# lisanhu/LongReadMapper

Hardware: AMD Instinct MI355X
Metric: aligned Gbp/sec (higher is better)
Workload: dtype u8/u64 integer; 1 GPU; E. coli K-12 sized synthetic reference (4641652 bp, 5% planted repeats), 100000 x 10000 bp ont-profile reads per GPU; seed_len=20, thres=300, gact_T=320, gact_O=120, gact_W=128, reads_per_gpu=100000, read_len=10000, streams=3, sa_sampled=1, parallelism=reads sharded, index replicated (1 RCCL bcast)

## Files before the change

### include/lrm_accel.h

```cpp
#ifndef LRM_ACCEL_H
#define LRM_ACCEL_H

#include <stdint.h>
#include <stddef.h>

#ifdef __cplusplus
extern "C" {
#endif

#define LRM_ABI_VERSION 3

typedef struct lrm_entry { uint64_t key, val, bucket; } lrm_entry;

typedef struct lrm_params { uint64_t batch_size; uint32_t seed_len, thres; } lrm_params;

typedef struct lrm_dna_fmi {
    uint64_t length, o_len, csa_len;
    uint64_t *c, *o, *csa;
    int o_ratio, csa_ratio;
    char *bwt;
} lrm_dna_fmi;

typedef struct lrm_lc_hash { uint64_t *lc; uint64_t len; int hlen; } lrm_lc_hash;

typedef struct lrm_ui40 { uint32_t low; uint8_t high; } lrm_ui40;
typedef struct lrm_sa_mem { uint64_t start, len; lrm_ui40 *mem; } lrm_sa_mem;

typedef struct lrm_mta_entry {
    uint64_t name_len; char *name; int name_own;
    uint64_t offset; size_t seq_len;
} lrm_mta_entry;

typedef struct lrm_seq_meta { uint64_t loc, off; int32_t seq_id; uint8_t strand; } lrm_seq_meta;

typedef struct lrm_cigar { uint8_t *cigar; int n_cigar_op; int score; } lrm_cigar;

typedef struct lrm_gact_params { int T, O, W; } lrm_gact_params;
#define LRM_GACT_T_DEFAULT 320
#define LRM_GACT_O_DEFAULT 120
#define LRM_GACT_W_DEFAULT 128

typedef struct lrm_index lrm_index;

typedef struct lrm_index_options {
    uint32_t struct_size;
    int32_t sa_sampled;
    int32_t lc_long;
    int32_t lc_long_max;
    int32_t lc_pair;
    uint32_t lcx_threshold;
    uint32_t lc_entry_bytes;
    int32_t lc_core;
    uint32_t lc_count_bits;
    int32_t seed_table;
    uint32_t seed_table_len;
    uint32_t seed_table_share;
    uint32_t seed_table_bits;
    uint32_t seed_table_count_bits;
    uint32_t reserved[2];
} lrm_index_options;
void lrm_index_options_init(lrm_index_options *o);

typedef struct lrm_map_options {
    uint32_t struct_size;
    int32_t dense_results;
    int32_t gact_impl;
    int32_t seed_rounds;
    int32_t vote_exact_only;
    uint32_t slice_reads;
    uint32_t sub_batches;
    uint32_t group_subs;
    uint32_t bs_waves;
    uint32_t cigar_text;
    uint32_t copy_threads;
    uint32_t keep_reads;
    uint32_t anchored;
    uint32_t anchor_min_len;
    uint32_t clip;
    uint32_t clip_penalty;
    uint32_t clip_end_bonus;
    uint32_t split;
    uint32_t split_min_len;
} lrm_map_options;
void lrm_map_options_init(lrm_map_options *o);

const char *lrm_last_error(void);
void lrm_free(void *p);
int lrm_abi_version(void);
int lrm_device_count(void);


uint64_t lrm_index_blob_bytes(uint64_t length, int hlen, int mta_len);

int lrm_index_pack_blob(const lrm_dna_fmi *fmi, const lrm_lc_hash *lch,
                        const lrm_sa_mem *sa, const char *content, uint64_t con_len,
                        const lrm_mta_entry *mta, int mta_len, void *blob, uint64_t blob_bytes);

int lrm_index_upload(lrm_index **out, const lrm_dna_fmi *fmi, const lrm_lc_hash *lch,
                     const lrm_sa_mem *sa, const char *content, uint64_t con_len,
                     const lrm_mta_entry *mta, int mta_len, int device);

int lrm_index_pack_device(const lrm_dna_fmi *fmi, const lrm_lc_hash *lch, const lrm_sa_mem *sa,
                          const char *content, uint64_t con_len, const lrm_mta_entry *mta, int mta_len,
                          void *d_blob, uint64_t blob_bytes, int device);

int lrm_index_upload_multi(lrm_index **out, const lrm_dna_fmi *fmi, const lrm_lc_hash *lch,
                           const lrm_sa_mem *sa, const char *content, uint64_t con_len,
                           const lrm_mta_entry *mta, int mta_len, const int *devices, int ngpus);
int lrm_index_replicas(const lrm_index *idx);
lrm_index *lrm_index_replica(lrm_index *idx, int r);

uint64_t lrm_index_blob_bytes_opt(uint64_t length, int hlen, int mta_len, const lrm_index_options *opt);
int lrm_index_pack_blob_opt(const lrm_dna_fmi *fmi, const lrm_lc_hash *lch, const lrm_sa_mem *sa, const char *content,
                            uint64_t con_len, const lrm_mta_entry *mta, int mta_len, void *blob, uint64_t blob_bytes,
                            const lrm_index_options *opt);
int lrm_index_pack_device_opt(const lrm_dna_fmi *fmi, const lrm_lc_hash *lch, const lrm_sa_mem *sa, const char *content,
                              uint64_t con_len, const lrm_mta_entry *mta, int mta_len, void *d_blob, uint64_t blob_bytes,
                              int device, const lrm_index_options *opt);
int lrm_index_upload_opt(lrm_index **out, const lrm_dna_fmi *fmi, const lrm_lc_hash *lch, const lrm_sa_mem *sa,
                         const char *content, uint64_t con_len, const lrm_mta_entry *mta, int mta_len,
                         const int *devices, int ngpus, const lrm_index_options *opt);
int lrm_index_adopt_device_opt(lrm_index **out, void *d_blob, uint64_t blob_bytes, int device, const lrm_index_options *opt);
int lrm_index_upload_blob_opt(lrm_index **out, const void *blob, uint64_t blob_bytes, int device, const lrm_index_options *opt);

int lrm_index_set_map_options(lrm_index *idx, const lrm_map_options *opt);

typedef struct lrm_index_tables {
    int32_t lc_long;
    int32_t lc_pair;
    int32_t lc_entry_bytes;
    int32_t lc_core;
    int32_t seed_table_len;
    int32_t seed_table_share;
    int32_t seed_table_bits;
    int32_t seed_table_slot_bytes;
    int32_t seed_table_count_bits;
    int32_t reserved0;
    uint64_t seed_table_side_entries;
    uint64_t derived_bytes;
    uint64_t reserved[4];
} lrm_index_tables;
int lrm_index_get_tables(const lrm_index *idx, lrm_index_tables *out);

int lrm_index_adopt_device(lrm_index **out, void *d_blob, uint64_t blob_bytes, int device);

int lrm_index_upload_blob(lrm_index **out, const void *blob, uint64_t blob_bytes, int device);

void lrm_index_free(lrm_index *idx);


int lrm_seed_batch(lrm_index *idx, const char *reads_buf, uint64_t stride,
                   const uint32_t *lens, uint64_t n, lrm_params p, lrm_entry *best_out);

int lrm_extend_batch(lrm_index *idx, char *reads_buf, uint64_t stride,
                     const uint32_t *lens, uint64_t n, const lrm_entry *best,
                     lrm_gact_params gp, lrm_cigar *cig_out, uint8_t *store_mem,
                     uint64_t store_stride, int *score_out, lrm_seq_meta *meta_out,
                     int *meta_r_out);

int lrm_map_batch(lrm_index *idx, char *reads_buf, uint64_t stride, const uint32_t *lens, uint64_t n,
                  lrm_params p, lrm_gact_params gp, lrm_entry *best_out, lrm_cigar *cig_out,
                  uint8_t *store_mem, uint64_t store_stride, int *score_out, lrm_seq_meta *meta_out,
                  int *meta_r_out);

typedef struct lrm_ticket lrm_ticket;
int lrm_map_batch_submit(lrm_index *idx, char *reads_buf, uint64_t stride, const uint32_t *lens, uint64_t n,
                         lrm_params p, lrm_gact_params gp, lrm_entry *best_out, lrm_cigar *cig_out,
                         uint8_t *store_mem, uint64_t store_stride, int *score_out, lrm_seq_meta *meta_out,
                         int *meta_r_out, const lrm_map_options *opt, lrm_ticket **ticket_out);
int lrm_map_batch_wait(lrm_ticket *ticket);

void *lrm_host_alloc(uint64_t bytes);
void lrm_host_free(void *p);
int lrm_host_register(void *p, uint64_t bytes);
int lrm_host_unregister(void *p);

int lrm_pair_end(int argc, const char *argv[]);

void lrm_result_flags(const int *score, const int *meta_r, const lrm_seq_meta *meta,
                      uint64_t n, int *flag_out, int *mapq_out, int *valid_out);

#define LRM_MAPQ_SLOTS 4096
#define LRM_MAPQ_OVERFLOW 1u
typedef struct lrm_mapq { uint32_t n1, n2, radius; uint8_t mapq, phase, flags, pad; } lrm_mapq;
void lrm_result_flags_mapq(const int *score, const int *meta_r, const lrm_seq_meta *meta, const lrm_mapq *mq, uint64_t n,
                           int *flag_out, int *mapq_out, int *valid_out);
int lrm_map_batch_submit_mapq(lrm_index *idx, char *reads_buf, uint64_t stride, const uint32_t *lens, uint64_t n,
                              lrm_params p, lrm_gact_params gp, lrm_entry *best_out, lrm_cigar *cig_out,
                              uint8_t *store_mem, uint64_t store_stride, int *score_out, lrm_seq_meta *meta_out,
                              int *meta_r_out, const lrm_map_options *opt, lrm_mapq *mapq_out, lrm_ticket **ticket_out);

typedef struct lrm_aln_summary {
    uint32_t n_eq, n_x, n_ins, n_del;
    uint32_t ins_runs, del_runs;
    uint32_t clip_left, clip_right;
} lrm_aln_summary;
void lrm_aln_summary_host(const uint8_t *ops, int n_ops, lrm_aln_summary *out);

typedef struct lrm_batch_extras {
    uint32_t struct_size, reserved;
    lrm_mapq *mapq_out;
    lrm_aln_summary *summary_out;
} lrm_batch_extras;
int lrm_map_batch_submit_ex(lrm_index *idx, char *reads_buf, uint64_t stride, const uint32_t *lens, uint64_t n,
                            lrm_params p, lrm_gact_params gp, lrm_entry *best_out, lrm_cigar *cig_out,
                            uint8_t *store_mem, uint64_t store_stride, int *score_out, lrm_seq_meta *meta_out,
                            int *meta_r_out, const lrm_map_options *opt, const lrm_batch_extras *ex, lrm_ticket **ticket_out);

typedef struct lrm_batch_diff {
    uint32_t struct_size, reserved;
    uint64_t *off_out;
    uint32_t *cnt_out;
    uint32_t *events_out;
    uint64_t cap;
    uint64_t *needed_out;
} lrm_batch_diff;
int lrm_map_batch_submit_ex2(lrm_index *idx, char *reads_buf, uint64_t stride, const uint32_t *lens, uint64_t n,
                             lrm_params p, lrm_gact_params gp, lrm_entry *best_out, lrm_cigar *cig_out,
                             uint8_t *store_mem, uint64_t store_stride, int *score_out, lrm_seq_meta *meta_out,
                             int *meta_r_out, const lrm_map_options *opt, const lrm_batch_extras *ex,
                             const lrm_batch_diff *diff, lrm_ticket **ticket_out);


typedef struct lrm_workspace lrm_workspace;

int lrm_workspace_create(lrm_workspace **out, lrm_index *idx, uint64_t n_max,
                         uint32_t max_len, uint32_t seed_len, uint32_t thres);
void lrm_workspace_free(lrm_workspace *ws);
uint64_t lrm_workspace_bytes(const lrm_workspace *ws);

int lrm_seed_batch_dev(lrm_index *idx, lrm_workspace *ws, const char *d_reads,
                       uint64_t stride, const uint32_t *d_lens, uint64_t n,
                       uint32_t max_len, lrm_params p, lrm_entry *d_best, void *stream);

int lrm_seed_batch_mapq_dev(lrm_index *idx, lrm_workspace *ws, const char *d_reads, uint64_t stride,
                            const uint32_t *d_lens, uint64_t n, uint32_t max_len, lrm_params p,
                            lrm_entry *d_best, lrm_mapq *d_mapq, void *stream);

int lrm_extend_batch_dev(lrm_index *idx, lrm_workspace *ws, char *d_reads, uint64_t stride,
                         const uint32_t *d_lens, uint64_t n, uint32_t max_len,
                         const lrm_entry *d_best, lrm_gact_params gp, uint8_t *d_store,
                         uint64_t store_stride, int32_t *d_n_ops, int32_t *d_score,
                         lrm_seq_meta *d_meta, int32_t *d_meta_r, void *stream);

#define LRM_ANCHOR_DIAGS 64
#define LRM_ANCHOR_ANCHORED 1u
#define LRM_ANCHOR_FALLBACK 2u
#define LRM_ANCHOR_NO_LEFT 4u
#define LRM_ANCHOR_LEFT_CLIPPED 8u
#define LRM_ANCHOR_RIGHT_CLIPPED 16u
#define LRM_ANCHOR_SOFT_LEFT 32u
#define LRM_ANCHOR_SOFT_RIGHT 64u
typedef struct lrm_anchor {
    uint64_t text_pos;
    uint32_t read_pos, len;
    int32_t delta;
    uint32_t left_ops;
    uint32_t flags;
} lrm_anchor;
int lrm_extend_batch_anchored_dev(lrm_index *idx, lrm_workspace *ws, char *d_reads, uint64_t stride,
                                  const uint32_t *d_lens, uint64_t n, uint32_t max_len,
                                  const lrm_entry *d_best, lrm_gact_params gp, uint8_t *d_store,
                                  uint64_t store_stride, int32_t *d_n_ops, int32_t *d_score,
                                  lrm_seq_meta *d_meta, int32_t *d_meta_r, lrm_anchor *d_anchor, uint32_t min_len,
                                  void *stream);

typedef struct lrm_clip { uint32_t left, right; } lrm_clip;
int lrm_extend_batch_clipped_dev(lrm_index *idx, lrm_workspace *ws, char *d_reads, uint64_t stride,
                                 const uint32_t *d_lens, uint64_t n, uint32_t max_len,
                                 const lrm_entry *d_best, lrm_gact_params gp, uint8_t *d_store,
                                 uint64_t store_stride, int32_t *d_n_ops, int32_t *d_score,
                                 lrm_seq_meta *d_meta, int32_t *d_meta_r, lrm_anchor *d_anchor, uint32_t min_len,
                                 uint32_t clip_penalty, uint32_t clip_end_bonus, lrm_clip *d_clip, void *stream);

int lrm_aln_summary_dev(lrm_index *idx, const uint8_t *d_store, uint64_t store_stride,
                        const int32_t *d_n_ops, const int32_t *d_score, const int32_t *d_meta_r,
                        uint64_t n, lrm_aln_summary *d_out, void *stream);

#define LRM_DIFF_X 0u
#define LRM_DIFF_D_OPEN 1u
#define LRM_DIFF_D_MORE 2u
#define LRM_DIFF_BASE(w) ((uint32_t) (w) & 0xFFu)
#define LRM_DIFF_KIND(w) (((uint32_t) (w) >> 8) & 3u)
#define LRM_DIFF_EQ_BEFORE(w) ((uint32_t) (w) >> 10)
int lrm_aln_diff_offsets_dev(const lrm_aln_summary *d_summary, uint64_t n, uint64_t *d_off, void *stream);
int lrm_aln_diff_dev(lrm_index *idx, const uint8_t *d_store, uint64_t store_stride, const int32_t *d_n_ops,
                     const int32_t *d_score, const int32_t *d_meta_r, const lrm_seq_meta *d_meta, uint64_t n,
                     const uint64_t *d_off, uint64_t cap, uint32_t *d_events, void *stream);
int64_t lrm_aln_diff_host(const uint8_t *ops, int n_ops, const uint8_t *target, uint64_t target_len, uint32_t *events_out);
int lrm_md_format(const uint32_t *events, uint64_t count, uint32_t n_eq, char *buf, int buflen);

#define LRM_SPLIT_MIN_DEFAULT 200
#define LRM_SEG_RIGHT 1u
#define LRM_SEG_ALIGNED 2u
typedef struct lrm_segment { uint32_t read, start, len, flags; } lrm_segment;

int lrm_split_plan(const uint32_t *lens, const lrm_clip *clip, uint64_t n, uint32_t split_min_len, lrm_segment *seg_out,
                   uint64_t cap, uint64_t *n_seg);
int lrm_clip_of_cigar(const lrm_cigar *cig, int is_text, uint32_t *left, uint32_t *right);

typedef struct lrm_split_dev {
    uint64_t cap;
    lrm_segment *seg;
    char *rows; uint64_t row_stride;
    uint32_t *lens;
    lrm_entry *best;
    uint8_t *store; uint64_t store_stride;
    int32_t *n_ops, *score;
    lrm_seq_meta *meta; int32_t *meta_r;
    lrm_anchor *anchor;
    lrm_clip *clip;
} lrm_split_dev;
int lrm_split_batch_dev(lrm_index *idx, lrm_workspace *ws_seg, const char *d_reads, uint64_t stride, const uint32_t *d_lens,
                        uint64_t n, const lrm_clip *d_clip, lrm_params p, lrm_gact_params gp, uint32_t anchor_min_len,
                        uint32_t clip_penalty, uint32_t clip_end_bonus, uint32_t split_min_len, const lrm_split_dev *out,
                        uint64_t *n_seg, void *stream);

typedef struct lrm_split_out {
    uint64_t cap, n_seg;
    lrm_segment *seg;
    char *rows; uint64_t row_stride;
    uint32_t *lens;
    lrm_entry *best;
    lrm_cigar *cig;
    uint8_t *store; uint64_t store_stride;
    int *score;
    lrm_seq_meta *meta; int *meta_r;
    lrm_anchor *anchor;
    lrm_clip *clip;
} lrm_split_out;
int lrm_split_batch(lrm_index *idx, const char *reads_buf, uint64_t stride, const uint32_t *lens, uint64_t n,
                    const lrm_cigar *cig, const lrm_seq_meta *meta, const int *meta_r, lrm_params p, lrm_gact_params gp,
                    const lrm_map_options *opt, lrm_split_out *out);

#define LRM_SEC_ALIGNED 1u
#define LRM_SEC_DUPLICATE 2u
typedef struct lrm_secondary { uint32_t read, hits, flags, pad; } lrm_secondary;
typedef struct lrm_secondary_options {
    uint32_t struct_size;
    uint32_t min_hits;
    uint32_t ratio_pct;
    uint32_t anchored;
    uint32_t anchor_min_len;
    uint32_t clip;
    uint32_t clip_penalty;
    uint32_t clip_end_bonus;
} lrm_secondary_options;

int lrm_rival_dev(lrm_index *idx, lrm_workspace *ws, const uint32_t *d_lens, uint64_t n, lrm_params p,
                  const lrm_entry *d_best, const lrm_mapq *d_mapq, uint32_t min_hits, uint32_t ratio_pct,
                  lrm_entry *d_rival, void *stream);
int lrm_rival_host(const uint64_t *keys, uint64_t n_keys, const lrm_entry *best, uint32_t len, uint32_t min_hits,
                   uint32_t ratio_pct, uint32_t slots, lrm_entry *out);
int lrm_secondary_plan(const lrm_mapq *mapq, uint64_t n, uint32_t min_hits, uint32_t ratio_pct, lrm_secondary *table,
                       uint64_t cap, uint64_t *n_sec);

typedef struct lrm_secondary_dev {
    uint64_t cap;
    lrm_secondary *table;
    char *rows; uint64_t row_stride;
    uint32_t *lens;
    lrm_entry *rival;
    uint8_t *store; uint64_t store_stride;
    int32_t *n_ops, *score;
    lrm_seq_meta *meta; int32_t *meta_r;
    lrm_anchor *anchor;
    lrm_clip *clip;
} lrm_secondary_dev;
int lrm_secondary_batch_dev(lrm_index *idx, lrm_workspace *ws, const char *d_reads, uint64_t stride, const uint32_t *d_lens,
                            uint64_t n, const lrm_entry *d_best, const lrm_mapq *d_mapq, const lrm_seq_meta *d_meta,
                            const int32_t *d_meta_r, lrm_params p, lrm_gact_params gp, const lrm_secondary_options *so,
                            const lrm_secondary_dev *out, uint64_t *n_sec, void *stream);

typedef struct lrm_secondary_out {
    uint64_t cap, n_sec;
    lrm_secondary *table;
    char *rows; uint64_t row_stride;
    uint32_t *lens;
    lrm_entry *rival;
    lrm_cigar *cig;
    uint8_t *store; uint64_t store_stride;
    int *score;
    lrm_seq_meta *meta; int *meta_r;
    lrm_anchor *anchor;
    lrm_clip *clip;
} lrm_secondary_out;
int lrm_secondary_batch(lrm_index *idx, const char *reads_buf, uint64_t stride, const uint32_t *lens, uint64_t n,
                        const lrm_mapq *mapq, const lrm_seq_meta *meta, const int *meta_r, lrm_params p, lrm_gact_params gp,
                        const lrm_map_options *opt, const lrm_secondary_options *so, lrm_secondary_out *out);

typedef struct lrm_stats {
    uint64_t vote_tier2_items;
    uint64_t vote_tier3_items;
    uint64_t reads_decided_phase0;
    uint64_t gact_tiles;
    uint64_t seeds_evaluated;
    uint64_t seed_table_lookups;
    uint64_t seed_rank_requests;
    uint64_t vote_redo_items;
    uint64_t bs_wave_tiles;
    uint64_t bs_pass1_pairs_masked;
    uint64_t bs_pass1_pairs_plain;
    uint64_t bs_blocks_full;
    uint64_t bs_blocks_windowed;
    uint64_t bs_blocks_skipped;
    uint64_t bs_refill_rounds;
} lrm_stats;
int lrm_workspace_set_counting(lrm_workspace *ws, int enable);
int lrm_workspace_stats(lrm_workspace *ws, lrm_stats *out, void *stream);

#define LRM_N_KERNELS 9
int lrm_workspace_set_timing(lrm_workspace *ws, int enable);
int lrm_workspace_timing(lrm_workspace *ws, double *ms, uint64_t *launches, void *stream);
const char *lrm_kernel_name(int kernel);

int lrm_debug_seed_search(lrm_index *idx, const char *read, uint32_t len, uint32_t seed_len,
                          uint32_t thres, int32_t *j_out, uint64_t *rr_out, uint64_t *k_out,
                          uint64_t *l_out, uint64_t cap, uint64_t *n_out);

int lrm_debug_vote_results(lrm_workspace *ws, uint64_t n, uint64_t *out, void *stream);

int lrm_debug_set_vote_limits(lrm_index *idx, uint32_t t3_limit, uint32_t t3_slots);

int lrm_debug_set_mapq_slots(lrm_index *idx, uint32_t slots);

int lrm_debug_reload_env(lrm_index *idx);

int lrm_debug_rccl_selftest(int device, uint64_t bytes);

int lrm_debug_anchor(lrm_index *idx, const char *read, uint32_t len, uint64_t loc, uint32_t min_len, lrm_anchor *out);

int lrm_debug_gact(const char *q, int n, const char *d, int m, lrm_gact_params gp,
                   uint8_t *ops, int *n_ops, int *score, int device);
int lrm_debug_gact_impl(const char *q, int n, const char *d, int m, lrm_gact_params gp, int impl,
                        uint8_t *ops, int *n_ops, int *score, int device);

typedef struct lrm_debug_gact_table {
    uint64_t n;
    const char *reads; uint64_t stride; const uint32_t *lens;
    const char *text; uint64_t text_len; const uint64_t *toffs; const uint32_t *tlens;
    const int32_t *meta_r;
    uint8_t *store; uint64_t store_stride; int32_t *n_ops; int32_t *score;
    uint64_t *counters;
} lrm_debug_gact_table;
int lrm_debug_gact_jobs(const lrm_debug_gact_table *t, lrm_gact_params gp, int impl, uint32_t bs_waves, int count, int device);

#ifdef __cplusplus
}
#endif
#endif
```

### longreadmapper_amd/capi.py

```python
import ctypes as C
import os

from . import _build
from .records import *

SYMBOLS = {
    "lrm_last_error": (C.c_char_p, []),
    "lrm_free": (None, [C.c_void_p]),
    "lrm_abi_version": (C.c_int, []),
    "lrm_device_count": (C.c_int, []),
    "lrm_index_blob_bytes": (C.c_uint64, [C.c_uint64, C.c_int, C.c_int]),
    "lrm_index_pack_blob": (C.c_int, [C.POINTER(DnaFmi), C.POINTER(LcHash), C.POINTER(SaMem), C.c_void_p,
                                      C.c_uint64, C.POINTER(MtaEntry), C.c_int, C.c_void_p, C.c_uint64]),
    "lrm_index_upload": (C.c_int, [C.POINTER(C.c_void_p), C.POINTER(DnaFmi), C.POINTER(LcHash),
                                   C.POINTER(SaMem), C.c_void_p, C.c_uint64, C.POINTER(MtaEntry), C.c_int, C.c_int]),
    "lrm_index_pack_device": (C.c_int, [C.POINTER(DnaFmi), C.POINTER(LcHash), C.POINTER(SaMem), C.c_void_p,
                                        C.c_uint64, C.POINTER(MtaEntry), C.c_int, C.c_void_p, C.c_uint64, C.c_int]),
    "lrm_index_options_init": (None, [C.POINTER(IndexOptions)]),
    "lrm_map_options_init": (None, [C.POINTER(MapOptions)]),
    "lrm_index_blob_bytes_opt": (C.c_uint64, [C.c_uint64, C.c_int, C.c_int, C.POINTER(IndexOptions)]),
    "lrm_index_pack_blob_opt": (C.c_int, [C.POINTER(DnaFmi), C.POINTER(LcHash), C.POINTER(SaMem), C.c_void_p,
                                          C.c_uint64, C.POINTER(MtaEntry), C.c_int, C.c_void_p, C.c_uint64,
                                          C.POINTER(IndexOptions)]),
    "lrm_index_pack_device_opt": (C.c_int, [C.POINTER(DnaFmi), C.POINTER(LcHash), C.POINTER(SaMem), C.c_void_p,
                                            C.c_uint64, C.POINTER(MtaEntry), C.c_int, C.c_void_p, C.c_uint64, C.c_int,
                                            C.POINTER(IndexOptions)]),
    "lrm_index_upload_opt": (C.c_int, [C.POINTER(C.c_void_p), C.POINTER(DnaFmi), C.POINTER(LcHash),
                                       C.POINTER(SaMem), C.c_void_p, C.c_uint64, C.POINTER(MtaEntry), C.c_int,
                                       C.POINTER(C.c_int), C.c_int, C.POINTER(IndexOptions)]),
    "lrm_index_adopt_device_opt": (C.c_int, [C.POINTER(C.c_void_p), C.c_void_p, C.c_uint64, C.c_int,
                                             C.POINTER(IndexOptions)]),
    "lrm_index_upload_blob_opt": (C.c_int, [C.POINTER(C.c_void_p), C.c_void_p, C.c_uint64, C.c_int,
                                            C.POINTER(IndexOptions)]),
    "lrm_index_set_map_options": (C.c_int, [C.c_void_p, C.POINTER(MapOptions)]),
    "lrm_index_get_tables": (C.c_int, [C.c_void_p, C.POINTER(IndexTables)]),
    "lrm_map_batch_submit": (C.c_int, [C.c_void_p, C.c_void_p, C.c_uint64, C.c_void_p, C.c_uint64, Params, GactParams,
                                       C.c_void_p, C.c_void_p, C.c_void_p, C.c_uint64, C.c_void_p, C.c_void_p, C.c_void_p,
                                       C.POINTER(MapOptions), C.POINTER(C.c_void_p)]),
    "lrm_map_batch_submit_mapq": (C.c_int, [C.c_void_p, C.c_void_p, C.c_uint64, C.c_void_p, C.c_uint64, Params, GactParams,
                                            C.c_void_p, C.c_void_p, C.c_void_p, C.c_uint64, C.c_void_p, C.c_void_p, C.c_void_p,
                                            C.POINTER(MapOptions), C.c_void_p, C.POINTER(C.c_void_p)]),
    "lrm_map_batch_submit_ex": (C.c_int, [C.c_void_p, C.c_void_p, C.c_uint64, C.c_void_p, C.c_uint64, Params, GactParams,
                                          C.c_void_p, C.c_void_p, C.c_void_p, C.c_uint64, C.c_void_p, C.c_void_p, C.c_void_p,
                                          C.POINTER(MapOptions), C.POINTER(BatchExtras), C.POINTER(C.c_void_p)]),
    "lrm_map_batch_submit_ex2": (C.c_int, [C.c_void_p, C.c_void_p, C.c_uint64, C.c_void_p, C.c_uint64, Params, GactParams,
                                           C.c_void_p, C.c_void_p, C.c_void_p, C.c_uint64, C.c_void_p, C.c_void_p, C.c_void_p,
                                           C.POINTER(MapOptions), C.POINTER(BatchExtras), C.POINTER(BatchDiff), C.POINTER(C.c_void_p)]),
    "lrm_map_batch_wait": (C.c_int, [C.c_void_p]),
    "lrm_aln_diff_offsets_dev": (C.c_int, [C.c_void_p, C.c_uint64, C.c_void_p, C.c_void_p]),
    "lrm_aln_diff_dev": (C.c_int, [C.c_void_p, C.c_void_p, C.c_uint64, C.c_void_p, C.c_void_p, C.c_void_p, C.c_void_p, C.c_uint64,
                                   C.c_void_p, C.c_uint64, C.c_void_p, C.c_void_p]),
    "lrm_aln_diff_host": (C.c_int64, [C.c_void_p, C.c_int, C.c_void_p, C.c_uint64, C.c_void_p]),
    "lrm_md_format": (C.c_int, [C.c_void_p, C.c_uint64, C.c_uint32, C.c_void_p, C.c_int]),
    "lrm_aln_summary_host": (None, [C.c_void_p, C.c_int, C.POINTER(AlnSummary)]),
    "lrm_aln_summary_dev": (C.c_int, [C.c_void_p, C.c_void_p, C.c_uint64, C.c_void_p, C.c_void_p, C.c_void_p, C.c_uint64,
                                      C.c_void_p, C.c_void_p]),
    "lrm_debug_reload_env": (C.c_int, [C.c_void_p]),
    "lrm_debug_set_vote_limits": (C.c_int, [C.c_void_p, C.c_uint32, C.c_uint32]),
    "lrm_debug_set_mapq_slots": (C.c_int, [C.c_void_p, C.c_uint32]),
    "lrm_debug_gact_impl": (C.c_int, [C.c_void_p, C.c_int, C.c_void_p, C.c_int, GactParams, C.c_int, C.c_void_p,
                                      C.POINTER(C.c_int), C.POINTER(C.c_int), C.c_int]),
    "lrm_debug_gact_jobs": (C.c_int, [C.POINTER(GactTable), GactParams, C.c_int, C.c_uint32, C.c_int, C.c_int]),
    "lrm_index_adopt_device": (C.c_int, [C.POINTER(C.c_void_p), C.c_void_p, C.c_uint64, C.c_int]),
    "lrm_index_upload_blob": (C.c_int, [C.POINTER(C.c_void_p), C.c_void_p, C.c_uint64, C.c_int]),
    "lrm_index_free": (None, [C.c_void_p]),
    "lrm_seed_batch": (C.c_int, [C.c_void_p, C.c_void_p, C.c_uint64, C.c_void_p, C.c_uint64, Params, C.c_void_p]),
    "lrm_extend_batch": (C.c_int, [C.c_void_p, C.c_void_p, C.c_uint64, C.c_void_p, C.c_uint64, C.c_void_p,
                                   GactParams, C.c_void_p, C.c_void_p, C.c_uint64, C.c_void_p, C.c_void_p,
                                   C.c_void_p]),
    "lrm_map_batch": (C.c_int, [C.c_void_p, C.c_void_p, C.c_uint64, C.c_void_p, C.c_uint64, Params, GactParams,
                                C.c_void_p, C.c_void_p, C.c_void_p, C.c_uint64, C.c_void_p, C.c_void_p, C.c_void_p]),
    "lrm_host_alloc": (C.c_void_p, [C.c_uint64]),
    "lrm_host_free": (None, [C.c_void_p]),
    "lrm_host_register": (C.c_int, [C.c_void_p, C.c_uint64]),
    "lrm_host_unregister": (C.c_int, [C.c_void_p]),
    "lrm_pair_end": (C.c_int, [C.c_int, C.c_void_p]),
    "lrm_index_upload_multi": (C.c_int, [C.POINTER(C.c_void_p), C.POINTER(DnaFmi), C.POINTER(LcHash),
                                         C.POINTER(SaMem), C.c_void_p, C.c_uint64, C.POINTER(MtaEntry), C.c_int,
                                         C.POINTER(C.c_int), C.c_int]),
    "lrm_index_replicas": (C.c_int, [C.c_void_p]),
    "lrm_index_replica": (C.c_void_p, [C.c_void_p, C.c_int]),
    "lrm_result_flags": (None, [C.c_void_p, C.c_void_p, C.c_void_p, C.c_uint64, C.c_void_p, C.c_void_p, C.c_void_p]),
    "lrm_result_flags_mapq": (None, [C.c_void_p, C.c_void_p, C.c_void_p, C.c_void_p, C.c_uint64, C.c_void_p, C.c_void_p,
                                     C.c_void_p]),
    "lrm_workspace_create": (C.c_int, [C.POINTER(C.c_void_p), C.c_void_p, C.c_uint64, C.c_uint32, C.c_uint32,
                                       C.c_uint32]),
    "lrm_workspace_free": (None, [C.c_void_p]),
    "lrm_workspace_bytes": (C.c_uint64, [C.c_void_p]),
    "lrm_seed_batch_dev": (C.c_int, [C.c_void_p, C.c_void_p, C.c_void_p, C.c_uint64, C.c_void_p, C.c_uint64,
                                     C.c_uint32, Params, C.c_void_p, C.c_void_p]),
    "lrm_seed_batch_mapq_dev": (C.c_int, [C.c_void_p, C.c_void_p, C.c_void_p, C.c_uint64, C.c_void_p, C.c_uint64,
                                          C.c_uint32, Params, C.c_void_p, C.c_void_p, C.c_void_p]),
    "lrm_extend_batch_dev": (C.c_int, [C.c_void_p, C.c_void_p, C.c_void_p, C.c_uint64, C.c_void_p, C.c_uint64,
                                       C.c_uint32, C.c_void_p, GactParams, C.c_void_p, C.c_uint64, C.c_void_p,
                                       C.c_void_p, C.c_void_p, C.c_void_p, C.c_void_p]),
    "lrm_extend_batch_anchored_dev": (C.c_int, [C.c_void_p, C.c_void_p, C.c_void_p, C.c_uint64, C.c_void_p, C.c_uint64,
                                                C.c_uint32, C.c_void_p, GactParams, C.c_void_p, C.c_uint64, C.c_void_p,
                                                C.c_void_p, C.c_void_p, C.c_void_p, C.c_void_p, C.c_uint32, C.c_void_p]),
    "lrm_extend_batch_clipped_dev": (C.c_int, [C.c_void_p, C.c_void_p, C.c_void_p, C.c_uint64, C.c_void_p, C.c_uint64,
                                               C.c_uint32, C.c_void_p, GactParams, C.c_void_p, C.c_uint64, C.c_void_p,
                                               C.c_void_p, C.c_void_p, C.c_void_p, C.c_void_p, C.c_uint32, C.c_uint32,
                                               C.c_uint32, C.c_void_p, C.c_void_p]),
    "lrm_split_plan": (C.c_int, [C.c_void_p, C.c_void_p, C.c_uint64, C.c_uint32, C.c_void_p, C.c_uint64, u64p]),
    "lrm_clip_of_cigar": (C.c_int, [C.POINTER(Cigar), C.c_int, u32p, u32p]),
    "lrm_split_batch_dev": (C.c_int, [C.c_void_p, C.c_void_p, C.c_void_p, C.c_uint64, C.c_void_p, C.c_uint64, C.c_void_p, Params,
                                      GactParams, C.c_uint32, C.c_uint32, C.c_uint32, C.c_uint32, C.POINTER(SplitDev), u64p,
                                      C.c_void_p]),
    "lrm_split_batch": (C.c_int, [C.c_void_p, C.c_void_p, C.c_uint64, C.c_void_p, C.c_uint64, C.c_void_p, C.c_void_p, C.c_void_p,
                                  Params, GactParams, C.POINTER(MapOptions), C.POINTER(SplitOut)]),
    "lrm_rival_dev": (C.c_int, [C.c_void_p, C.c_void_p, C.c_void_p, C.c_uint64, Params, C.c_void_p, C.c_void_p, C.c_uint32, C.c_uint32,
                                C.c_void_p, C.c_void_p]),
    "lrm_rival_host": (C.c_int, [C.c_void_p, C.c_uint64, C.POINTER(Entry), C.c_uint32, C.c_uint32, C.c_uint32, C.c_uint32,
                                 C.POINTER(Entry)]),
    "lrm_secondary_plan": (C.c_int, [C.c_void_p, C.c_uint64, C.c_uint32, C.c_uint32, C.c_void_p, C.c_uint64, u64p]),
    "lrm_secondary_batch_dev": (C.c_int, [C.c_void_p, C.c_void_p, C.c_void_p, C.c_uint64, C.c_void_p, C.c_uint64, C.c_void_p, C.c_void_p,
                                          C.c_void_p, C.c_void_p, Params, GactParams, C.POINTER(SecondaryOptions),
                                          C.POINTER(SecondaryDev), u64p, C.c_void_p]),
    "lrm_secondary_batch": (C.c_int, [C.c_void_p, C.c_void_p, C.c_uint64, C.c_void_p, C.c_uint64, C.c_void_p, C.c_void_p, C.c_void_p,
                                      Params, GactParams, C.POINTER(MapOptions), C.POINTER(SecondaryOptions), C.POINTER(SecondaryOut)]),
    "lrm_accaln_secondary": (C.c_int, [C.c_char_p, C.c_char_p, C.c_char_p, Params, GactParams, C.c_int, C.c_long, u64p, u64p,
                                       C.POINTER(MapOptions), C.POINTER(SecondaryOptions)]),
    "lrm_debug_anchor": (C.c_int, [C.c_void_p, C.c_void_p, C.c_uint32, C.c_uint64, C.c_uint32, C.POINTER(Anchor)]),
    "lrm_workspace_stats": (C.c_int, [C.c_void_p, C.POINTER(Stats), C.c_void_p]),
    "lrm_debug_vote_results": (C.c_int, [C.c_void_p, C.c_uint64, C.c_void_p, C.c_void_p]),
    "lrm_workspace_set_counting": (C.c_int, [C.c_void_p, C.c_int]),
    "lrm_workspace_set_timing": (C.c_int, [C.c_void_p, C.c_int]),
    "lrm_workspace_timing": (C.c_int, [C.c_void_p, C.c_void_p, C.c_void_p, C.c_void_p]),
    "lrm_kernel_name": (C.c_char_p, [C.c_int]),
    "lrm_debug_seed_search": (C.c_int, [C.c_void_p, C.c_void_p, C.c_uint32, C.c_uint32, C.c_uint32, C.c_void_p,
                                        C.c_void_p, C.c_void_p, C.c_void_p, C.c_uint64, u64p]),
    "lrm_debug_rccl_selftest": (C.c_int, [C.c_int, C.c_uint64]),
    "lrm_debug_gact": (C.c_int, [C.c_void_p, C.c_int, C.c_void_p, C.c_int, GactParams, C.c_void_p,
                                 C.POINTER(C.c_int), C.POINTER(C.c_int), C.c_int]),
    "lrm_cat_from_seqs": (C.c_int, [C.POINTER(C.c_char_p), C.POINTER(C.c_char_p), u64p, C.c_int, C.c_uint64,
                                    C.POINTER(C.c_void_p), u64p, C.POINTER(C.POINTER(MtaEntry))]),
    "lrm_sa_build": (C.c_int, [C.c_void_p, C.c_uint64, C.c_void_p]),
    "lrm_host_index_build": (C.c_int, [C.c_void_p, C.c_uint64, C.POINTER(MtaEntry), C.c_int, C.c_int, C.c_int,
                                       C.POINTER(HostIndex)]),
    "lrm_host_index_free": (None, [C.POINTER(HostIndex)]),
    "lrm_host_index_write": (C.c_int, [C.POINTER(HostIndex), C.c_char_p]),
    "lrm_host_index_read": (C.c_int, [C.c_char_p, C.POINTER(HostIndex)]),
    "lrm_fmi_write": (C.c_int, [C.POINTER(DnaFmi), C.c_char_p]),
    "lrm_fmi_read": (C.c_int, [C.POINTER(DnaFmi), C.c_char_p]),
    "lrm_lc_write": (C.c_int, [C.c_char_p, C.POINTER(LcHash)]),
    "lrm_lc_read": (C.c_int, [C.c_char_p, C.POINTER(LcHash)]),
    "lrm_sa5_write": (C.c_int, [C.c_char_p, C.c_void_p, C.c_uint64]),
    "lrm_sa5_read": (C.c_int64, [C.c_char_p, C.c_void_p, C.c_uint64]),
    "lrm_mta_write": (C.c_int, [C.c_char_p, C.POINTER(MtaEntry), C.c_int]),
    "lrm_mta_read": (C.c_int, [C.c_char_p, C.POINTER(C.POINTER(MtaEntry))]),
    "lrm_mta_free": (None, [C.POINTER(MtaEntry), C.c_int]),
    "lrm_accidx": (C.c_int, [C.c_char_p, C.c_int, C.c_int, C.c_uint64]),
    "lrm_reader_open": (C.c_int, [C.POINTER(C.c_void_p), C.c_char_p]),
    "lrm_reader_next": (C.c_int64, [C.c_void_p, C.c_uint64, C.POINTER(ReadBatch)]),
    "lrm_reader_next_into": (C.c_int64, [C.c_void_p, C.c_uint64, C.POINTER(ReadBatch), C.c_void_p, C.c_uint64]),
    "lrm_read_batch_free": (None, [C.POINTER(ReadBatch)]),
    "lrm_reader_close": (None, [C.c_void_p]),
    "lrm_parse_cigar": (C.c_int, [C.c_void_p, C.c_int, C.c_void_p, C.c_int]),
    "lrm_sam_header": (C.c_void_p, [C.POINTER(MtaEntry), C.c_int, C.c_long, u64p]),
    "lrm_sam_format": (C.c_void_p, [C.POINTER(ReadBatch), C.POINTER(MtaEntry), C.c_int, C.c_void_p, C.c_void_p,
                                    C.c_void_p, C.c_void_p, C.c_uint64, u64p]),
    "lrm_sam_format_split": (C.c_void_p, [C.POINTER(ReadBatch), C.POINTER(MtaEntry), C.c_int, C.c_void_p, C.c_void_p, C.c_void_p,
                                          C.c_void_p, C.c_uint64, C.c_int, C.c_int, C.POINTER(SplitOut), u64p]),
    "lrm_sam_format_mapq": (C.c_void_p, [C.POINTER(ReadBatch), C.POINTER(MtaEntry), C.c_int, C.c_void_p, C.c_void_p, C.c_void_p,
                                         C.c_void_p, C.c_uint64, C.c_int, C.c_int, C.POINTER(SplitOut), C.c_void_p, u64p]),
    "lrm_sam_format_md": (C.c_void_p, [C.POINTER(ReadBatch), C.POINTER(MtaEntry), C.c_int, C.c_void_p, C.c_void_p, C.c_void_p,
                                       C.c_void_p, C.c_uint64, C.c_int, C.c_int, C.POINTER(SplitOut), C.c_void_p, C.c_void_p,
                                       C.c_void_p, C.c_void_p, C.c_void_p, u64p]),
    "lrm_sam_format_secondary": (C.c_void_p, [C.POINTER(ReadBatch), C.POINTER(MtaEntry), C.c_int, C.c_void_p, C.c_void_p, C.c_void_p,
                                              C.c_void_p, C.c_uint64, C.c_int, C.c_int, C.POINTER(SplitOut), C.c_void_p, C.c_void_p,
                                              C.c_void_p, C.c_void_p, C.c_void_p, C.POINTER(SecondaryOut), u64p]),
    "lrm_accaln_md": (C.c_int, [C.c_char_p, C.c_char_p, C.c_char_p, Params, GactParams, C.c_int, C.c_long, u64p, u64p,
                                C.POINTER(MapOptions), C.c_int, C.c_int]),
    "lrm_paf_format": (C.c_void_p, [C.POINTER(ReadBatch), C.POINTER(MtaEntry), C.c_int, C.c_void_p, C.c_void_p, C.c_void_p,
                                    C.c_void_p, C.c_uint64, C.c_int, C.c_void_p, C.c_void_p, u64p]),
    "lrm_accaln_paf": (C.c_int, [C.c_char_p, C.c_char_p, C.c_char_p, Params, GactParams, C.c_int, u64p, u64p,
                                 C.POINTER(MapOptions), C.c_int]),
    "lrm_accaln": (C.c_int, [C.c_char_p, C.c_char_p, C.c_char_p, Params, GactParams, C.c_int, C.c_long, u64p, u64p]),
    "lrm_accaln_opt": (C.c_int, [C.c_char_p, C.c_char_p, C.c_char_p, Params, GactParams, C.c_int, C.c_long, u64p, u64p,
                                 C.POINTER(MapOptions)]),
    "lrm_accaln_mapq": (C.c_int, [C.c_char_p, C.c_char_p, C.c_char_p, Params, GactParams, C.c_int, C.c_long, u64p, u64p,
                                  C.POINTER(MapOptions), C.c_int]),
}


def _load():
    try:
        import torch
    except Exception:
        pass
    path = _build.ACCEL_LIB
    if not os.path.exists(path):
        path = _build.build_accel()
    lib = C.CDLL(path)
    for name, (res, args) in SYMBOLS.items():
        fn = getattr(lib, name)
        fn.restype = res
        fn.argtypes = args
    return lib


lib = _load()


def index_options(**kw):
    o = IndexOptions()
    lib.lrm_index_options_init(C.byref(o))
    for k, v in kw.items():
        if k not in _INDEX_OPTION_NAMES:
            raise AttributeError("lrm_index_options has no field %r" % k)
        if v is not None:
            setattr(o, k, v)
    return o


_INDEX_OPTION_NAMES = frozenset(n for n, _ in IndexOptions._fields_) - {"struct_size", "reserved"}


def map_options(**kw):
    o = MapOptions()
    lib.lrm_map_options_init(C.byref(o))
    for k, v in kw.items():
        if v is not None:
            getattr(o, k)
            setattr(o, k, v)
    return o


class LrmError(RuntimeError):
    pass


def failure(what="", **fields):
    e = LrmError("%s: %s" % (what or "liblrm_accel", lib.lrm_last_error().decode(errors="replace")))
    e.__dict__.update(fields)
    return e


def check(rc, what=""):
    if rc < 0:
        raise failure(what)
    return rc
```

### longreadmapper_amd/csrc/lrm_internal.h

```cpp
#pragma once
#include <stddef.h>
#include <stdint.h>
#include <stdlib.h>
#include <string.h>
#include "../../include/lrm_accel.h"

#define LRM_BLOB_MAGIC 0x4c524d424c4f4232ull
#define LRM_OCC_ROWS 64

struct LrmOccEntry {
    uint64_t cnt;
    uint64_t mask;
};
struct LrmOccBlock { LrmOccEntry sym[4]; };
static_assert(sizeof(LrmOccBlock) == 64, "occ block must be one 64-B line");

struct LrmMtaDev { uint64_t offset, seq_len; };

struct LrmBlobHeader {
    uint64_t magic, version;
    uint64_t length;
    uint64_t c4[4];
    uint64_t dollar_row;
    uint64_t n_blocks;
    uint64_t lc_entries;
    uint64_t sa_len, con_len;
    uint64_t off_occ, off_lc, off_sa, off_content, off_mta;
    uint64_t total_bytes;
    int32_t hlen, mta_len;
    uint64_t off_lcx, n_lcx;
    uint64_t sa_ratio;
    uint64_t reserved[10];
};
static_assert(sizeof(LrmBlobHeader) == 256, "header is 256 B");

struct LrmIndexView {
    const LrmOccBlock *occ;
    const uint64_t *lc;
    const uint64_t *lcx;
    uint64_t n_lcx;
    const uint64_t *sa;
    const char *content;
    const LrmMtaDev *mta;
    uint64_t length, dollar_row, sa_len, con_len;
    uint64_t c4[4];
    int32_t hlen, mta_len;
    const uint64_t *lcl;
    int32_t hl;
    int32_t sa_shift;
    int32_t lcl_pair;
    int32_t lcl_kbits;
    const uint64_t *core;
    const uint64_t *lclx;
    uint64_t lclx_mask;
    const uint64_t *sd;
    const uint64_t *sdx;
    uint64_t sdx_mask;
    int32_t sd_len;
    int32_t sd_f;
    int32_t sd_bits;
    int32_t sd_kbits;
    int32_t sd_slot;
    int32_t sd_cbits;
};

struct LrmEnv {
    static constexpr int MAXV = 32;
    const char *name[MAXV];
    long long val[MAXV];
    int n;
    bool get(const char *key, long long *out) const;
};
void lrm_env_snapshot(LrmEnv *e);
struct LrmIndexTune {
    int sa_ratio;
    int lc_long, lc_long_max, lc_pair, lc_entry_bytes, lc_count_bits, lc_core;
    int sd, sd_len, sd_f, sd_bits, sd_cbits;
    uint64_t lcx_threshold;
};
struct LrmMapTune {
    int dense, gact_impl, seed_rounds, cigar_text, keep_reads, anchored;
    uint32_t anchor_min_len;
    uint32_t clip, clip_penalty, clip_end_bonus;
    uint32_t split, split_min_len;
    uint32_t slice_reads, sub_batches, group_subs, bs_waves, copy_threads;
    uint32_t ss_items, ss_lds_pad, vote_vg, vote_t1, vote_u, vote_load, vote_fast;
    uint32_t t3_limit, t3_slots;
    int ext_streams, seed_streams, verbose;
};
void lrm_resolve_index_tune(const lrm_index_options *opt, const LrmEnv &env, LrmIndexTune *out);
void lrm_resolve_map_tune(const lrm_map_options *opt, const LrmEnv &env, LrmMapTune *out);
template <typename T>
static inline void lrm_options_over_defaults(T *o, const T *opt) {
    if (opt) memcpy(o, opt, opt->struct_size && opt->struct_size < sizeof(T) ? opt->struct_size : sizeof(T));
}
template <typename T>
static inline void lrm_options_take_fields(T *o, const T *opt, size_t from, size_t to) {
    if (opt && opt->struct_size >= to) memcpy((char *) o + from, (const char *) opt + from, to - from);
}

struct LrmHostCtx;
struct lrm_index;
void lrm_call_map_tune(const lrm_index *ix, const lrm_map_options *opt, LrmMapTune *out);
struct lrm_index {
    void *d_blob;
    uint64_t blob_bytes;
    int owns_blob;
    int device;
    LrmBlobHeader hdr;
    LrmIndexView view;
    uint64_t *d_lcl;
    uint64_t *d_lclx;
    uint64_t *d_core;
    uint64_t *d_sd, *d_sdx;
    uint64_t sd_side_entries;
    uint64_t *d_cpl;
    int cpl_ok;
    uint64_t *d_sas;
    LrmHostCtx *host;
    int n_peers;
    lrm_index **peers;
    LrmEnv env;
    LrmIndexTune itune;
    LrmMapTune mtune;
    uint32_t dbg_t3_limit, dbg_t3_slots;
    uint32_t dbg_mapq_slots;
};

struct LrmPhaseRes {
    uint64_t key1, val1, bucket1;
    uint64_t key2, val2, bucket2;
};

struct LrmDevCounters {
    unsigned long long bs_queue;
    unsigned long long vote_ticket[2];
    unsigned long long seed_traffic[3];
    unsigned long long reserved[2];
    unsigned long long decided_phase0;
    unsigned long long gact_tiles;
    unsigned long long pad[2];
    unsigned long long vote_fast_ticket[2];
    unsigned long long vote_redo_n[2];
    unsigned long long vote_big_n[2];
    unsigned long long vote_big_ticket[2];
    unsigned long long bs_count[7];
};
enum { LRM_BSC_WAVE_TILES = 0, LRM_BSC_P1_MASKED, LRM_BSC_P1_PLAIN, LRM_BSC_P2_FULL, LRM_BSC_P2_WINDOWED, LRM_BSC_P2_SKIPPED,
       LRM_BSC_REFILLS, LRM_BSC_N };
static_assert(offsetof(LrmDevCounters, decided_phase0) == 64 && sizeof(LrmDevCounters) == 216, "counters are addressed by the device as laid out here");
#define LRM_ERR_VOTE_OVERFLOW 1u
#define LRM_VOTE_T1_LIMIT 192
#ifndef LRM_VOTE_T3_SLOTS
#define LRM_VOTE_T3_SLOTS 1024
#endif
#define LRM_VOTE_T3_LIMIT (LRM_VOTE_T3_SLOTS * 3 / 4)
#define LRM_VOTE_GRID 1536
#ifndef LRM_VOTE_FAST_GRID
#define LRM_VOTE_FAST_GRID 1792
#endif
#define LRM_VOTE_KC_CAP 16384

enum LrmKernelId { LRM_K_PACK2BIT = 0, LRM_K_SEED_SEARCH, LRM_K_VOTE, LRM_K_DECIDE,
                   LRM_K_LOCUS, LRM_K_REVCOMP, LRM_K_GACT, LRM_K_PACK_PLANAR, LRM_K_GACT_BS,
                   LRM_K_COUNT };
#define LRM_MAX_TIMED 4096

struct LrmBsScratch {
    uint64_t *qpl; uint64_t wpr;
    uint32_t *rflags;
    uint32_t *ckpt;
    uint64_t *codes; uint64_t cw;
    int32_t *ncodes;
};

#define LRM_WS_SEED 1
#define LRM_WS_EXTEND 2
struct lrm_workspace {
    lrm_index *idx;
    int parts;
    int timing;
    int counting;
    int n_timed;
    void *ev_start[LRM_MAX_TIMED], *ev_stop[LRM_MAX_TIMED];
    int ev_kernel[LRM_MAX_TIMED];
    int device;
    uint64_t n_max;
    uint64_t n_last;
    uint32_t max_len, seed_len, thres;
    uint32_t P;
    uint32_t cap_q;
    uint64_t words_per_read;
    uint64_t bytes;
    uint64_t *d_reads2;
    uint64_t *d_rec;
    uint32_t *d_recq;
    uint32_t *d_cnt;
    uint64_t *d_kc_key;
    uint32_t *d_kc_ord;
    uint64_t *d_redo;
    uint64_t *d_big;
    uint64_t *d_gtab;
    uint32_t *d_glock;
    uint32_t g_slices, g_slots;
    LrmPhaseRes *d_phase;
    uint8_t *d_decided;
    uint32_t *d_hcount;
    LrmDevCounters *d_counters;
    uint64_t hist_n;
    volatile uint32_t *h_err;
    uint32_t *d_err;
    LrmBsScratch bs;
    struct LrmAnchorScratch *an;
    struct LrmSplitScratch *sp;
    uint8_t *d_mq_phase;
    struct LrmSecScratch *sec;
};

int lrm_lcl_prepare_index(lrm_index *idx);

void lrm_set_error(const char *fmt, ...);
#define LRM_LOCAL __attribute__((visibility("hidden")))

static inline int base_code(char c) {
    switch (c) { case 'A': return 0; case 'C': return 1; case 'G': return 2; case 'T': return 3; default: return -1; }
}

static_assert(sizeof(lrm_ui40) == 8, "ui40 is 8 bytes in RAM (sa_use.h:17-20)");
static inline uint64_t ui40_get(const lrm_ui40 &v) { return ((uint64_t) v.high << 32) | v.low; }
static inline void ui40_put(lrm_ui40 *slot, uint64_t v) { *reinterpret_cast<uint64_t *>(slot) = v; }

template <typename T>
static inline bool lrm_alloc(T *&p, uint64_t n, const char *what, bool zero = false) {
    const size_t bytes = (size_t) (n ? n : 1) * sizeof(T);
    p = (T *) (zero ? calloc(1, bytes) : malloc(bytes));
    if (!p) lrm_set_error("out of memory (%s, %llu bytes)", what, (unsigned long long) bytes);
    return p != nullptr;
}
int lrm_host_threads(void);
int lrm_require_device(int device);
int lrm_workspace_create_parts(lrm_workspace **out, lrm_index *idx, uint64_t n_max, uint32_t max_len, uint32_t seed_len,
                               uint32_t thres, int parts);
int lrm_ws_take_error(lrm_workspace *ws);
void lrm_host_ctx_free(lrm_index *idx);
void lrm_time_begin(lrm_workspace *ws, int kernel, void *stream);
void lrm_time_end(lrm_workspace *ws, void *stream);

int lrm_index_make_handle(lrm_index **out, void *d_blob, uint64_t bytes, int device, int owns, const LrmBlobHeader &h,
                          const lrm_index_options *opt);
int lrm_index_upload_one(lrm_index **out, const lrm_dna_fmi *fmi, const lrm_lc_hash *lch, const lrm_sa_mem *sa, const char *content,
                         uint64_t con_len, const lrm_mta_entry *mta, int mta_len, int device, const lrm_index_options *opt);

int lrm_launch_pack_rows(const uint8_t *d_src, uint64_t pitch, uint64_t row_cap, const uint32_t *d_len, const uint64_t *d_off,
                         uint8_t *d_dense, uint64_t rows, void *stream);
int lrm_launch_cigar_text(const uint8_t *d_store, uint64_t pitch, const int32_t *d_n_ops, const int32_t *d_score, const int32_t *d_meta_r,
                          uint32_t *d_tlen, const uint64_t *d_off, uint8_t *d_dense, uint64_t rows, void *stream);
int lrm_launch_aln_summary(const uint8_t *d_store, uint64_t pitch, const int32_t *d_n_ops, const int32_t *d_score, const int32_t *d_meta_r,
                           uint64_t rows, lrm_aln_summary *d_out, void *stream);
int lrm_launch_aln_diff(const uint8_t *d_store, uint64_t pitch, const int32_t *d_n_ops, const int32_t *d_score, const int32_t *d_meta_r,
                        const lrm_seq_meta *d_meta, const char *d_content, uint64_t con_len, uint64_t rows, const uint64_t *d_off,
                        uint64_t cap, uint32_t *d_events, void *stream);
int lrm_launch_aln_diff_offsets(const lrm_aln_summary *d_sum, uint64_t rows, uint64_t *d_off, void *stream);
int lrm_launch_seed(lrm_index *idx, lrm_workspace *ws, const char *d_reads, uint64_t stride,
                    const uint32_t *d_lens, uint64_t n, uint32_t seed_len,
                    uint32_t thres, lrm_entry *d_best, const LrmMapTune &mt, void *stream, uint8_t *d_phase_out = nullptr);
struct LrmVoteLaunch {
    const uint8_t *decided;
    uint64_t n; uint32_t seed_len; int phase_lo, phase_hi;
    uint32_t tbits;
    int round;
    const LrmMapTune *mt;
};
int lrm_launch_vote(lrm_index *idx, lrm_workspace *ws, const LrmVoteLaunch &v, void *stream);
uint8_t *lrm_mapq_phase_buf(lrm_workspace *ws);
int lrm_launch_mapq(lrm_index *idx, lrm_workspace *ws, const uint32_t *d_lens, uint64_t n, uint32_t seed_len, uint32_t thres,
                    const lrm_entry *d_best, lrm_mapq *d_mapq, void *stream);
int lrm_wait_event(void *ev);
int lrm_launch_debug_seed(lrm_index *idx, const char *d_read, uint32_t len, uint32_t seed_len,
                          uint64_t *d_reads2, uint64_t words, int32_t *d_j, uint64_t *d_rr,
                          uint64_t *d_k, uint64_t *d_l, uint64_t cap, void *stream);
```

### longreadmapper_amd/csrc/vote_kernels.hip

```cpp
#include <hip/hip_runtime.h>
#include "vote_hits.h"

#define VG 16
#define VG_MAX 64
#define T1_SLOTS 256
#define T1_LIMIT LRM_VOTE_T1_LIMIT
#define T3_SLOTS LRM_VOTE_T3_SLOTS
#define T3_LIMIT LRM_VOTE_T3_LIMIT
#define T3_CHUNK 256

#define EMPTY_KEY 0x8000000000000000ull

__device__ __forceinline__ uint32_t bucket_hash(uint64_t bucket) {
    uint32_t x = (uint32_t) bucket ^ (uint32_t) (bucket >> 29);
    x *= 0x9E3779B1u;
    x ^= x >> 15;
    return x * 0x85EBCA6Bu;
}

struct VoteTable {
    uint64_t *key;
    uint64_t *cf;
    uint32_t slots;
};

template <int NT>
__device__ __forceinline__ void table_clear(const VoteTable &t, uint32_t tid) {
    for (uint32_t s = tid; s < t.slots; s += NT) { t.key[s] = EMPTY_KEY; t.cf[s] = 0; }
}

__device__ __forceinline__ void slot_count(const VoteTable &t, uint32_t slot, bool lower, uint64_t key, uint32_t order, uint32_t n) {
    if (lower) atomicMin((unsigned long long *) &t.key[slot], (unsigned long long) key);
    uint32_t *cf = reinterpret_cast<uint32_t *>(&t.cf[slot]);
    atomicAdd(cf + 1, n);
    atomicMax(cf, 0xFFFFFFFFu - order);
}

__device__ __forceinline__ bool vote_insert(const VoteTable &t, uint64_t key, uint32_t order, uint32_t hash, uint32_t n = 1u) {
    const uint64_t bucket = key >> 4;
    uint32_t slot = (uint32_t) (((uint64_t) hash * t.slots) >> 32);
    for (uint32_t probe = 0; probe < t.slots; ++probe) {
        const unsigned long long prev = atomicCAS((unsigned long long *) &t.key[slot], EMPTY_KEY, key);
        if (prev == EMPTY_KEY || (prev >> 4) == bucket) {
            slot_count(t, slot, prev != EMPTY_KEY && key < prev, key, order, n);
            return true;
        }
        slot = slot + 1 == t.slots ? 0 : slot + 1;
    }
    return false;
}

__device__ __forceinline__ bool vote_admit(const VoteTable &t, uint64_t key, uint32_t order, uint32_t passes, uint32_t pass) {
    const uint32_t hash = bucket_hash(key >> 4);
    if (passes == 1 || (hash >> 16) % passes == pass) return vote_insert(t, key, order, hash);
    return true;
}

struct TopEntry { uint64_t key, bucket; uint32_t val, first; };
struct PhaseTop { TopEntry a, b; };

__device__ __forceinline__ void write_phase(LrmPhaseRes *out, const PhaseTop &p) {
    LrmPhaseRes res = {0, 0, 0, 0, 0, 0};
    if (p.a.val) { res.key1 = p.a.key; res.val1 = p.a.val; res.bucket1 = p.a.bucket; }
    if (p.b.val) { res.key2 = p.b.key; res.val2 = p.b.val; res.bucket2 = p.b.bucket; }
    *out = res;
}

struct Top2 { uint64_t k1, k2; uint32_t s1, s2; };

template <int NT, bool GLOBAL = false>
__device__ __forceinline__ Top2 table_top2(const VoteTable &t, uint32_t tid) {
    uint64_t k1 = 0, k2 = 0;
    uint32_t s1 = 0, s2 = 0;
    for (uint32_t s = tid; s < t.slots; s += NT) {
        const uint64_t k = GLOBAL ? __hip_atomic_load(&t.cf[s], __ATOMIC_RELAXED, __HIP_MEMORY_SCOPE_AGENT) : t.cf[s];
        if (k > k1) { k2 = k1; s2 = s1; k1 = k; s1 = s; }
        else if (k > k2) { k2 = k; s2 = s; }
    }
    const uint64_t m1 = wave_max_u64(k1);
    const bool win = k1 == m1 && (m1 >> 32) != 0;
    const uint64_t m2 = wave_max_u64(win ? k2 : k1);
    Top2 r;
    r.k1 = (m1 >> 32) ? m1 : 0; r.k2 = (m2 >> 32) ? m2 : 0; r.s1 = 0; r.s2 = 0;
    if (r.k1) {
        const unsigned long long b = __ballot(k1 == m1);
        r.s1 = (uint32_t) __builtin_amdgcn_readlane((int) s1, (int) __builtin_ctzll(b));
    }
    if (r.k2) {
        const bool has = (win ? k2 : k1) == m2;
        const unsigned long long b = __ballot(has);
        const int src = (int) __builtin_ctzll(b);
        r.s2 = (uint32_t) __builtin_amdgcn_readlane((int) (win ? s2 : s1), src);
    }
    return r;
}

__device__ __forceinline__ TopEntry entry_of(const VoteTable &t, uint64_t k, uint32_t s, bool global = false) {
    TopEntry e = {0, 0, 0, 0};
    if (k) {
        e.key = global ? __hip_atomic_load(&t.key[s], __ATOMIC_RELAXED, __HIP_MEMORY_SCOPE_AGENT) : t.key[s];
        e.bucket = e.key >> 4; e.val = (uint32_t) (k >> 32); e.first = 0xFFFFFFFFu - (uint32_t) k;
    }
    return e;
}
__device__ __forceinline__ PhaseTop phase_of(const VoteTable &t, uint64_t k1, uint32_t s1, uint64_t k2, uint32_t s2, bool global = false) {
    return PhaseTop{entry_of(t, k1, s1, global), entry_of(t, k2, s2, global)};
}

__device__ __forceinline__ Top2 block_top2(const Top2 *s_top) {
    Top2 r = {0, 0, 0, 0};
    for (int x = 0; x < 4; ++x) {
        const Top2 c = s_top[x];
        const uint64_t ks[2] = {c.k1, c.k2};
        const uint32_t ss[2] = {c.s1, c.s2};
        for (int y = 0; y < 2; ++y) {
            if (ks[y] > r.k1) { r.k2 = r.k1; r.s2 = r.s1; r.k1 = ks[y]; r.s1 = ss[y]; }
            else if (ks[y] > r.k2) { r.k2 = ks[y]; r.s2 = ss[y]; }
        }
    }
    return r;
}

__device__ __forceinline__ uint32_t table_slots_for(uint32_t x, uint32_t load, uint32_t cap) {
    const uint32_t eff = x * 100u / load + 64;
    return eff < cap ? eff : cap;
}

struct VoteItems {
    uint64_t n;
    uint32_t P, np, phase_lo, cap_q, tbits, load;
    LrmPhaseRes *phase_res;
};
struct Item { const uint64_t *rec; const uint32_t *recq; uint32_t cnt, H, iter; LrmPhaseRes *out; };

struct ItemId { uint64_t read, id; uint32_t iter; };
__device__ __forceinline__ ItemId item_decode(uint64_t item, const VoteItems &v) {
    ItemId r;
    r.read = item / v.np;
    r.iter = v.phase_lo + (uint32_t) (item - r.read * v.np);
    r.id = r.read * (uint64_t) v.P + r.iter;
    return r;
}

template <int NT, int VOTE_U>
__device__ __forceinline__ bool vote_hits(const LrmIndexView &ix, const VoteTable &t, const Staged &g, uint32_t tid, uint32_t passes,
                                          uint32_t pass, uint64_t *kc_key = nullptr, uint32_t *kc_ord = nullptr) {
    bool ok = true;
    for_each_hit<NT, VOTE_U>(ix, g, tid, [&](bool live, uint32_t h, uint64_t key, uint32_t order) __attribute__((always_inline)) {
        if (!live) return;
        if (kc_key) { kc_key[h] = key; kc_ord[h] = order; }
        ok &= vote_admit(t, key, order, passes, pass);
    });
    return ok;
}

struct WaveLds {
    uint64_t key[T1_SLOTS];
    uint64_t srec[T1_LIMIT / 2];
    uint64_t cf[T1_SLOTS];
    uint32_t off[T1_LIMIT / 2 + 4];
    uint32_t sq[T1_LIMIT / 2];
};

template <int VOTE_U>
__device__ __forceinline__ void vote_item_wave(const LrmIndexView &ix, const VoteItems &v, const Item &it, uint32_t lane, WaveLds &L) {
    const VoteTable t = {L.key, L.cf, table_slots_for(it.H, v.load, T1_SLOTS)};
    constexpr int NU = (T1_LIMIT + 63) / 64;
    uint64_t e[NU], sv[NU];
    uint32_t qq[NU];
#pragma unroll
    for (int u = 0; u < NU; ++u) {
        const uint32_t s = (uint32_t) u * 64 + lane;
        e[u] = s < it.cnt ? it.rec[s] : 0ull;
        qq[u] = s < it.cnt ? it.recq[s] : 0u;
    }
    table_clear<64>(t, lane);
#pragma unroll
    for (int u = 0; u < NU; ++u) sv[u] = (uint32_t) (e[u] >> 40) == 1 ? sa_of_unique(ix, e[u]) : 0ull;
    WaveStage st = {0, 0};
#pragma unroll
    for (int u = 0; u < NU; ++u) st = stage_repeats_wave(L.off, L.srec, L.sq, e[u], qq[u], st, lane);
#pragma unroll
    for (int u = 0; u < NU; ++u)
        if ((uint32_t) (e[u] >> 40) == 1) vote_admit(t, sv[u] - (uint64_t) (it.iter + qq[u] * v.P), qq[u] << v.tbits, 1u, 0u);
    if (st.n) vote_hits<64, VOTE_U>(ix, t, Staged{L.off, L.srec, L.sq, st.n, st.hits, it.iter, v.P, v.tbits}, lane, 1u, 0u);
    __builtin_amdgcn_fence(__ATOMIC_ACQ_REL, "wavefront");
    __builtin_amdgcn_wave_barrier();

    const Top2 w = table_top2<64>(t, lane);
    if (lane == 0) write_phase(it.out, phase_of(t, w.k1, w.s1, w.k2, w.s2));
    __builtin_amdgcn_wave_barrier();
}

struct BlockLds {
    uint64_t key[T3_SLOTS];
    uint64_t srec[T3_CHUNK];
    uint64_t cf[T3_SLOTS];
    uint32_t off[T3_CHUNK + 4];
    uint32_t sq[T3_CHUNK];
};
union VoteLds { WaveLds w[4]; BlockLds b; };

struct KeyScratch { uint64_t *key; uint32_t *ord; uint32_t cap; };
struct GlobalPool { uint64_t *tab; uint32_t *lock; uint32_t slices, slots; uint32_t *s_slice; };

template <int VOTE_U>
__device__ __forceinline__ void vote_item_block(const LrmIndexView &ix, const VoteItems &v, const Item &it, uint32_t slots, uint32_t limit,
                                                BlockLds &L, uint32_t *s_wsum, Top2 *s_top, uint32_t *err_word, const KeyScratch &kc,
                                                const GlobalPool &gp) {
    const uint32_t tid = threadIdx.x, wave = tid >> 6, lane = tid & 63u;
    const uint32_t H = it.H, cnt = it.cnt;
    VoteTable t = {L.key, L.cf, slots};
    uint32_t passes = (H + limit - 1) / limit;
    const bool big = gp.tab != nullptr && H > kc.cap && 2ull * H <= (uint64_t) gp.slots;
    if (big) {
        if (tid == 0) {
            uint32_t got = 0xFFFFFFFFu;
            for (uint32_t spin = 0; got == 0xFFFFFFFFu; ++spin) {
                const uint32_t sl = (blockIdx.x + spin) % gp.slices;
                if (atomicCAS(&gp.lock[sl], 0u, 1u) == 0u) got = sl;
                else __builtin_amdgcn_s_sleep(32);
            }
            *gp.s_slice = got;
        }
        __syncthreads();
        uint32_t gs = 1024;
        while (gs < 2 * H) gs <<= 1;
        uint64_t *base = gp.tab + (uint64_t) (*gp.s_slice) * 2ull * gp.slots;
        t.key = base; t.cf = base + gp.slots; t.slots = gs;
        passes = 1;
    }
    const bool cache = passes > 2 && H <= kc.cap;
    if (!big) t.slots = table_slots_for(passes > 1 ? limit : H, v.load, slots);
    PhaseTop best = {};
    for (uint32_t pass = 0; pass < passes; ++pass) {
        table_clear<256>(t, tid);
        if (big) { __threadfence(); __syncthreads(); }
        bool ok = true;
        if (cache && pass > 0) {
            __syncthreads();
            for (uint32_t i = tid; i < H; i += 256) ok &= vote_admit(t, kc.key[i], kc.ord[i], passes, pass);
        } else {
        uint32_t kbase = 0;
        for (uint32_t c0 = 0; c0 < cnt; c0 += T3_CHUNK) {
            const uint32_t nc = cnt - c0 < (uint32_t) T3_CHUNK ? cnt - c0 : (uint32_t) T3_CHUNK;
            const uint64_t e0 = tid < nc ? it.rec[c0 + tid] : 0ull;
            const uint32_t q0 = tid < nc ? it.recq[c0 + tid] : 0u;
            const uint32_t r0 = (uint32_t) (e0 >> 40);
            const uint64_t v0 = r0 == 1 ? sa_of_unique(ix, e0) : 0ull;
            const BlockStage st = stage_repeats_block<true>(L.off, L.srec, L.sq, s_wsum, e0, q0, r0);
            if (r0 == 1) {
                const uint64_t key = v0 - (uint64_t) (it.iter + q0 * v.P);
                if (cache) { const uint32_t i = kbase + st.urank; kc.key[i] = key; kc.ord[i] = q0 << v.tbits; }
                ok &= vote_admit(t, key, q0 << v.tbits, passes, pass);
            }
            if (st.nbig) ok &= vote_hits<256, VOTE_U>(ix, t, Staged{L.off, L.srec, L.sq, st.nbig, st.total, it.iter, v.P, v.tbits}, tid, passes, pass,
                                                      cache ? kc.key + kbase + st.nuni : nullptr, cache ? kc.ord + kbase + st.nuni : nullptr);
            kbase += st.nuni + st.total;
        }
        if (cache) __threadfence_block();
        }
        if (!ok) *(volatile uint32_t *) err_word = LRM_ERR_VOTE_OVERFLOW;
        if (big) __threadfence();
        __syncthreads();
        const Top2 w = big ? table_top2<256, true>(t, tid) : table_top2<256>(t, tid);
        if (lane == 0) s_top[wave] = w;
        __syncthreads();
        if (tid == 0) {
            const Top2 c = block_top2(s_top);
            auto rank = [](const TopEntry &e) { return e.val ? ((uint64_t) e.val << 32) | (0xFFFFFFFFu - e.first) : 0ull; };
            const uint64_t cks[2] = {c.k1, c.k2};
            const uint32_t css[2] = {c.s1, c.s2};
            PhaseTop nb = best;
            uint64_t r1 = rank(best.a), r2 = rank(best.b);
            for (int x = 0; x < 2; ++x) {
                const uint64_t ck = cks[x];
                if (!ck) continue;
                const TopEntry e = entry_of(t, ck, css[x], big);
                if (ck > r1) { nb.b = nb.a; r2 = r1; nb.a = e; r1 = ck; }
                else if (ck > r2) { nb.b = e; r2 = ck; }
            }
            best = nb;
        }
        __syncthreads();
    }
    if (tid == 0) write_phase(it.out, best);
    if (big) {
        __syncthreads();
        if (tid == 0) { __threadfence(); atomicExch(&gp.lock[*gp.s_slice], 0u); }
    }
}

#define FAST_SK_WORDS 512
#define FB_LIMIT 1536

#define EMPTY_ID 0x80000000u
#define FAST_NONE 0xFFFFFFFFu
struct FastTable { uint32_t *ident, *count; uint32_t slots; };
template <int NT>
__device__ __forceinline__ void table_clear(const FastTable &t, uint32_t tid) {
    for (uint32_t s = tid; s < t.slots; s += NT) { t.ident[s] = EMPTY_ID; t.count[s] = 0; }
}

__device__ __forceinline__ bool key_wide(uint64_t key) { return (uint32_t) (key >> 32) + 1u > 8u; }
__device__ __forceinline__ uint64_t bucket_of_ident(uint32_t id) {
    return id < 0x80000000u ? (uint64_t) id : (0x0FFFFFFF00000000ull | id);
}

__device__ __forceinline__ uint32_t fast_insert(const FastTable &t, uint32_t id, uint32_t hash) {
    uint32_t slot = (uint32_t) (((uint64_t) hash * t.slots) >> 32);
    for (uint32_t probe = 0; probe < t.slots; ++probe) {
        const uint32_t prev = atomicCAS(&t.ident[slot], EMPTY_ID, id);
        if (prev == EMPTY_ID || prev == id) { atomicAdd(&t.count[slot], 1u); return slot; }
        slot = slot + 1 == t.slots ? 0 : slot + 1;
    }
    return FAST_NONE;
}
__device__ __forceinline__ uint32_t fast_find(const FastTable &t, uint32_t id, uint32_t hash) {
    uint32_t slot = (uint32_t) (((uint64_t) hash * t.slots) >> 32);
    for (uint32_t probe = 0; probe < t.slots; ++probe) {
        const uint32_t prev = t.ident[slot];
        if (prev == EMPTY_ID) return FAST_NONE;
        if (prev == id) return slot;
        slot = slot + 1 == t.slots ? 0 : slot + 1;
    }
    return FAST_NONE;
}

#ifndef LRM_VOTE_FAST_LIST
#define LRM_VOTE_FAST_LIST 64
#endif
#define FAST_LIST LRM_VOTE_FAST_LIST
#define FB_LIST 512
__device__ __forceinline__ uint32_t hit_word(uint32_t slot, uint64_t key) { return (slot << 4) | ((uint32_t) key & 15u); }

template <int NT, int VOTE_U>
__device__ __forceinline__ void fast_hits(const LrmIndexView &ix, const FastTable &t, const Staged &g, uint32_t *sketch, uint32_t sk_mask,
                                          uint32_t tid, uint64_t *list, uint32_t cap, uint32_t &n_list, uint32_t *list_n, bool &wide) {
    for_each_hit<NT, VOTE_U>(ix, g, tid, [&](bool live, uint32_t, uint64_t key, uint32_t order) __attribute__((always_inline)) {
        uint32_t hw = FAST_NONE, oinv = 0;
        if (live) {
            const uint32_t hash = bucket_hash(key >> 4);
            wide |= key_wide(key);
            const uint32_t slot = fast_find(t, (uint32_t) (key >> 4), hash);
            if (slot != FAST_NONE) {
                atomicAdd(&t.count[slot], 1u);
                hw = hit_word(slot, key);
                oinv = 0xFFFFFFFFu - order;
            } else {
                const uint32_t c = (hash >> 5) & sk_mask;
                atomicAdd(&sketch[c >> 1], 1u << (16 * (c & 1)));
            }
        }
        const unsigned long long bm = __ballot(hw != FAST_NONE);
        if (bm) {
            uint32_t base;
            if (NT == 64) { base = n_list; n_list += (uint32_t) __popcll(bm); }
            else {
                uint32_t b0 = 0;
                if ((tid & 63u) == 0) b0 = atomicAdd(list_n, (uint32_t) __popcll(bm));
                base = (uint32_t) __builtin_amdgcn_readfirstlane((int) b0);
            }
            if (hw != FAST_NONE) {
                const uint32_t i = base + mask_rank(bm);
                if (i < cap) list[i] = ((uint64_t) oinv << 32) | hw;
            }
        }
    });
}

struct RankTop { uint64_t r; uint32_t s; };
__device__ __forceinline__ RankTop wave_top_rank(const RankTop &x) {
    const uint32_t hi = (uint32_t) (x.r >> 32), lo = (uint32_t) x.r;
    const uint32_t mh = wave_max_u32(hi);
    const uint32_t ml = wave_max_u32(hi == mh ? lo : 0u);
    RankTop w = {0, 0};
    if (mh) {
        const unsigned long long b = __ballot(hi == mh && lo == ml);
        w.r = ((uint64_t) mh << 32) | ml;
        w.s = (uint32_t) __builtin_amdgcn_readlane((int) x.s, (int) __builtin_ctzll(b));
    }
    return w;
}
template <int N>
__device__ __forceinline__ RankTop lane_top_rank(const uint64_t (&hr)[N], const uint32_t (&hw)[N], uint32_t skip) {
    RankTop b = {0, 0};
#pragma unroll
    for (int k = 0; k < N; ++k) {
        const uint32_t s = hw[k] >> 4;
        if (hr[k] > b.r && s != skip) { b.r = hr[k]; b.s = s; }
    }
    return b;
}
template <int N>
__device__ __forceinline__ uint32_t lane_low4_mask(const uint64_t (&hr)[N], const uint32_t (&hw)[N], const RankTop &a, const RankTop &b) {
    uint32_t m = 0;
#pragma unroll
    for (int k = 0; k < N; ++k) {
        const uint32_t s = hw[k] >> 4, bit = 0x8000u >> (hw[k] & 15u);
        if (hr[k] && s == a.s) m |= bit << 16;
        else if (hr[k] && b.r && s == b.s) m |= bit;
    }
    return m;
}
__device__ __forceinline__ TopEntry fast_entry(const FastTable &t, const RankTop &w, uint32_t mask16) {
    TopEntry e = {0, 0, 0, 0};
    if (w.r) {
        e.bucket = bucket_of_ident(t.ident[w.s]);
        e.key = (e.bucket << 4) | (uint32_t) (__clz((int) mask16) - 16);
        e.val = (uint32_t) (w.r >> 32); e.first = 0xFFFFFFFFu - (uint32_t) w.r;
    }
    return e;
}

template <int NT, int NL, int N>
__device__ __forceinline__ void list_ranks(const FastTable &t, const uint64_t *list, uint32_t n_list, uint32_t cap, uint32_t tid,
                                           uint64_t (&hr)[N], uint32_t (&hw)[N]) {
#pragma unroll
    for (int l = 0; l < NL; ++l) {
        const uint32_t i = (uint32_t) l * NT + tid;
        hr[N - NL + l] = 0; hw[N - NL + l] = FAST_NONE;
        if (i < n_list && i < cap) {
            const uint64_t x = list[i];
            hw[N - NL + l] = (uint32_t) x;
            hr[N - NL + l] = ((uint64_t) t.count[(uint32_t) x >> 4] << 32) | (x >> 32);
        }
    }
}
template <int NT, int WORDS>
__device__ __forceinline__ uint32_t sketch_max(const uint32_t *sketch, uint32_t tid) {
    static_assert(WORDS % NT == 0, "every thread scans WORDS / NT words");
    uint32_t m = 0;
#pragma unroll
    for (uint32_t s = 0; s < WORDS / NT; ++s) {
        const uint32_t x = sketch[s * NT + tid];
        const uint32_t lo = x & 0xffffu, hi = x >> 16;
        m = lo > m ? lo : m;
        m = hi > m ? hi : m;
    }
    return wave_max_u32(m);
}

struct FastLds {
    uint32_t ident[T1_SLOTS];
    uint32_t count[T1_SLOTS];
    uint64_t srec[64];
    uint64_t list[FAST_LIST];
    uint32_t off[64 + 4];
    uint32_t sq[64];
    uint32_t sketch[FAST_SK_WORDS];
};

#ifndef LRM_VOTE_FAST_WAVES
#define LRM_VOTE_FAST_WAVES (LRM_VOTE_FAST_GRID / 256)
#endif
#define FAST_CH 16
template <int VOTE_U>
__global__ __launch_bounds__(256) __attribute__((amdgpu_waves_per_eu(LRM_VOTE_FAST_WAVES, LRM_VOTE_FAST_WAVES)))
void vote_fast_kernel(LrmIndexView ix, const uint64_t *__restrict__ rec, const uint32_t *__restrict__ recq, const uint32_t *__restrict__ gcnt,
                      const uint32_t *__restrict__ ghits, const uint8_t *__restrict__ decided, VoteItems v, unsigned long long *ticket, uint64_t *__restrict__ redo, unsigned long long *redo_n,
                      uint64_t *__restrict__ big, unsigned long long *big_n) {
    __shared__ FastLds lds[4];
    const uint32_t lane = threadIdx.x & 63u;
    FastLds &L = lds[threadIdx.x >> 6];
    const uint64_t n_items = v.n * (uint64_t) v.np;
    constexpr int NU = (T1_LIMIT + 63) / 64;
    constexpr int NL = (FAST_LIST + 63) / 64;
    for (;;) {
        unsigned long long base = 0;
        if (lane == 0) base = atomicAdd(ticket, (unsigned long long) FAST_CH);
        base = ((unsigned long long) (uint32_t) __builtin_amdgcn_readfirstlane((int) (uint32_t) (base >> 32)) << 32) |
               (uint32_t) __builtin_amdgcn_readfirstlane((int) (uint32_t) base);
        if (base >= n_items) break;
        ItemId ii = item_decode(base, v);
        for (uint32_t it = 0; it < FAST_CH && base + it < n_items; ++it, ++ii.iter) {
            if (ii.iter == v.phase_lo + v.np) { ii.iter = v.phase_lo; ++ii.read; }
            const uint64_t item = base + it;
            const uint32_t iter = ii.iter;
            const uint64_t id = ii.read * (uint64_t) v.P + iter;
            if (decided && decided[ii.read]) continue;
            const uint32_t H = ghits[id], cnt = gcnt[id];
            if (H == 0) {
                if (lane == 0) { LrmPhaseRes z = {0, 0, 0, 0, 0, 0}; v.phase_res[id] = z; }
                continue;
            }
            if (cnt > (uint32_t) T1_LIMIT) {
                if (lane == 0) {
                    if (cnt <= (uint32_t) FB_LIMIT) big[atomicAdd(big_n, 1ull)] = item;
                    else redo[atomicAdd(redo_n, 1ull)] = item;
                }
                continue;
            }
            const FastTable t = {L.ident, L.count, table_slots_for(cnt, v.load, T1_SLOTS)};
            uint64_t e[NU], sv[NU];
            uint32_t qq[NU];
            const uint64_t *irec = rec + id * v.cap_q;
            const uint32_t *iq = recq + id * v.cap_q;
#pragma unroll
            for (int u = 0; u < NU; ++u) {
                const uint32_t s = (uint32_t) u * 64 + lane;
                e[u] = s < cnt ? irec[s] : 0ull;
                qq[u] = s < cnt ? iq[s] : 0u;
            }
            table_clear<64>(t, lane);
            unsigned long long any_big = 0;
#pragma unroll
            for (int u = 0; u < NU; ++u) {
                const uint32_t rr = (uint32_t) (e[u] >> 40);
                sv[u] = rr == 1 ? sa_of_unique(ix, e[u]) : 0ull;
                any_big |= __ballot(rr > 1);
            }
            if (any_big) {
#pragma unroll
                for (uint32_t s = 0; s < FAST_SK_WORDS / 64; ++s) L.sketch[s * 64 + lane] = 0;
            }
            __builtin_amdgcn_fence(__ATOMIC_RELEASE, "wavefront");
            __builtin_amdgcn_wave_barrier();
            uint64_t hr[NU + NL];
            uint32_t hw[NU + NL];
            bool wide = false;
#pragma unroll
            for (int u = 0; u < NU; ++u) {
                hw[u] = FAST_NONE;
                if ((uint32_t) (e[u] >> 40) == 1) {
                    const uint64_t key = sv[u] - (uint64_t) (iter + qq[u] * v.P);
                    wide |= key_wide(key);
                    const uint32_t slot = fast_insert(t, (uint32_t) (key >> 4), bucket_hash(key >> 4));
                    if (slot != FAST_NONE) hw[u] = hit_word(slot, key);
                }
            }
            __builtin_amdgcn_fence(__ATOMIC_ACQ_REL, "wavefront");
            __builtin_amdgcn_wave_barrier();
            uint32_t n_list = 0;
            if (any_big) {
#pragma unroll
                for (int u = 0; u < NU; ++u) {
                    if (__ballot((uint32_t) (e[u] >> 40) > 1) == 0) continue;
                    const WaveStage st = stage_repeats_wave(L.off, L.srec, L.sq, e[u], qq[u], WaveStage{0, 0}, lane);
                    fast_hits<64, VOTE_U>(ix, t, Staged{L.off, L.srec, L.sq, st.n, st.hits, iter, v.P, v.tbits}, L.sketch, 2 * FAST_SK_WORDS - 1, lane,
                                          L.list, (uint32_t) FAST_LIST, n_list, nullptr, wide);
                    __builtin_amdgcn_fence(__ATOMIC_ACQ_REL, "wavefront");
                    __builtin_amdgcn_wave_barrier();
                }
            }
            bool lost = wide;
#pragma unroll
            for (int u = 0; u < NU; ++u) {
                const bool uniq = (uint32_t) (e[u] >> 40) == 1;
                lost |= uniq && hw[u] == FAST_NONE;
                hr[u] = uniq && hw[u] != FAST_NONE ? ((uint64_t) t.count[hw[u] >> 4] << 32) | (0xFFFFFFFFu - (qq[u] << v.tbits)) : 0ull;
            }
            list_ranks<64, NL>(t, L.list, n_list, (uint32_t) FAST_LIST, lane, hr, hw);
            const RankTop a = wave_top_rank(lane_top_rank(hr, hw, FAST_NONE));
            const RankTop b = wave_top_rank(lane_top_rank(hr, hw, a.r ? a.s : FAST_NONE));
            const uint32_t lowm = wave_or_u32(lane_low4_mask(hr, hw, a, b));
            bool settled = n_list <= (uint32_t) FAST_LIST && __ballot(lost) == 0;
            if (any_big) settled = settled && sketch_max<64, FAST_SK_WORDS>(L.sketch, lane) < (uint32_t) (b.r >> 32);
            if (lane == 0) {
                if (settled) write_phase(&v.phase_res[id], PhaseTop{fast_entry(t, a, lowm >> 16), fast_entry(t, b, lowm & 0xffffu)});
                else redo[atomicAdd(redo_n, 1ull)] = item;
            }
            __builtin_amdgcn_wave_barrier();
        }
    }
}

#define FB_SLOTS 2048
#define FB_SK_WORDS 2048
struct FastBlockLds {
    uint32_t ident[FB_SLOTS];
    uint32_t count[FB_SLOTS];
    uint64_t srec[T3_CHUNK];
    uint64_t list[FB_LIST];
    uint32_t off[T3_CHUNK + 4];
    uint32_t sq[T3_CHUNK];
    uint32_t sketch[FB_SK_WORDS];
};
__device__ __forceinline__ RankTop block_top_rank(const RankTop *s_rk) {
    RankTop r = {0, 0};
    for (int x = 0; x < 4; ++x) if (s_rk[x].r > r.r) r = s_rk[x];
    return r;
}
template <int VOTE_U>
__global__ __launch_bounds__(256) __attribute__((amdgpu_waves_per_eu(3, 3)))
void vote_fast_block_kernel(LrmIndexView ix, const uint64_t *__restrict__ rec, const uint32_t *__restrict__ recq,
                            const uint32_t *__restrict__ gcnt, VoteItems v, unsigned long long *ticket, const uint64_t *__restrict__ big,
                            const unsigned long long *__restrict__ big_n, uint64_t *__restrict__ redo, unsigned long long *redo_n) {
    __shared__ FastBlockLds L;
    __shared__ uint32_t s_wsum[8], s_m[4], s_or[4], s_list_n;
    __shared__ RankTop s_rk[2][4];
    __shared__ unsigned long long s_at;
    const uint32_t tid = threadIdx.x, wave = tid >> 6, lane = tid & 63u;
    const uint64_t n_big = (uint64_t) *big_n;
    constexpr int NU = FB_LIMIT / 256;
    constexpr int NL = FB_LIST / 256;
    for (;;) {
        if (tid == 0) { s_at = atomicAdd(ticket, 1ull); s_list_n = 0; }
        __syncthreads();
        const uint64_t at = s_at;
        if (at >= n_big) break;
        const uint64_t item = big[at];
        const ItemId ii = item_decode(item, v);
        const uint64_t id = ii.id;
        const uint32_t iter = ii.iter, cnt = gcnt[id];
        const uint64_t *irec = rec + id * v.cap_q;
        const uint32_t *iq = recq + id * v.cap_q;
        const FastTable t = {L.ident, L.count, table_slots_for(cnt, v.load, FB_SLOTS)};
        table_clear<256>(t, tid);
        __syncthreads();
        bool ok = true;
        uint32_t any_big = 0;
        uint64_t hr[NU + NL];
        uint32_t hw[NU + NL], ho[NU];
#pragma unroll
        for (int k = 0; k < NU; ++k) {
            const uint32_t s = (uint32_t) k * 256 + tid;
            hw[k] = FAST_NONE; ho[k] = 0;
            const uint64_t e0 = s < cnt ? irec[s] : 0ull;
            const uint32_t r0 = (uint32_t) (e0 >> 40);
            any_big |= r0 > 1 ? 1u : 0u;
            if (r0 == 1) {
                const uint32_t q0 = iq[s];
                const uint64_t key = sa_of_unique(ix, e0) - (uint64_t) (iter + q0 * v.P);
                const uint32_t slot = fast_insert(t, (uint32_t) (key >> 4), bucket_hash(key >> 4));
                ok &= slot != FAST_NONE && !key_wide(key);
                if (slot != FAST_NONE) { hw[k] = hit_word(slot, key); ho[k] = 0xFFFFFFFFu - (q0 << v.tbits); }
            }
        }
        const bool block_big = __syncthreads_or((int) any_big) != 0;
        if (block_big) {
            for (uint32_t s = tid; s < FB_SK_WORDS; s += 256) L.sketch[s] = 0;
            uint32_t unused = 0;
            bool wide = false;
            for (uint32_t c0 = 0; c0 < cnt; c0 += 256) {
                const uint64_t e0 = c0 + tid < cnt ? irec[c0 + tid] : 0ull;
                const uint32_t q0 = c0 + tid < cnt ? iq[c0 + tid] : 0u;
                const uint32_t r0 = (uint32_t) (e0 >> 40);
                const BlockStage st = stage_repeats_block<false>(L.off, L.srec, L.sq, s_wsum, e0, q0, r0);
                if (st.nbig) fast_hits<256, VOTE_U>(ix, t, Staged{L.off, L.srec, L.sq, st.nbig, st.total, iter, v.P, v.tbits}, L.sketch, 2 * FB_SK_WORDS - 1, tid,
                                                    L.list, (uint32_t) FB_LIST, unused, &s_list_n, wide);
                __syncthreads();
            }
            ok &= !wide;
        }
        const uint32_t n_list = s_list_n;
#pragma unroll
        for (int k = 0; k < NU; ++k)
            hr[k] = hw[k] != FAST_NONE ? ((uint64_t) t.count[hw[k] >> 4] << 32) | ho[k] : 0ull;
        list_ranks<256, NL>(t, L.list, n_list, (uint32_t) FB_LIST, tid, hr, hw);
        const RankTop wa = wave_top_rank(lane_top_rank(hr, hw, FAST_NONE));
        if (lane == 0) s_rk[0][wave] = wa;
        __syncthreads();
        const RankTop a = block_top_rank(s_rk[0]);
        const RankTop wb = wave_top_rank(lane_top_rank(hr, hw, a.r ? a.s : FAST_NONE));
        if (lane == 0) s_rk[1][wave] = wb;
        __syncthreads();
        const RankTop b = block_top_rank(s_rk[1]);
        const uint32_t lowm = wave_or_u32(lane_low4_mask(hr, hw, a, b));
        const uint32_t m = block_big ? sketch_max<256, FB_SK_WORDS>(L.sketch, tid) : 0u;
        if (lane == 0) { s_or[wave] = lowm; s_m[wave] = m; }
        const bool all_ok = __syncthreads_and((int) ok) != 0;
        if (tid == 0) {
            uint32_t M = 0, lm = 0;
            for (int x = 0; x < 4; ++x) { M = s_m[x] > M ? s_m[x] : M; lm |= s_or[x]; }
            const bool settled = all_ok && n_list <= (uint32_t) FB_LIST && (!block_big || M < (uint32_t) (b.r >> 32));
            if (settled) write_phase(&v.phase_res[id], PhaseTop{fast_entry(t, a, lm >> 16), fast_entry(t, b, lm & 0xffffu)});
            else redo[atomicAdd(redo_n, 1ull)] = item;
        }
        __syncthreads();
    }
}

#ifndef LRM_VOTE_WAVES_PER_EU
#define LRM_VOTE_WAVES_PER_EU 6
#endif
template <int VOTE_U>
__global__ __launch_bounds__(256) __attribute__((amdgpu_waves_per_eu(LRM_VOTE_WAVES_PER_EU, LRM_VOTE_WAVES_PER_EU)))
void vote_kernel(LrmIndexView ix, const uint64_t *__restrict__ rec, const uint32_t *__restrict__ recq, const uint32_t *__restrict__ gcnt,
                 const uint32_t *__restrict__ ghits, const uint8_t *__restrict__ decided, VoteItems v, uint32_t slots3, uint32_t limit3, uint32_t vg, uint32_t limit1, unsigned long long *ticket,
                 uint64_t *__restrict__ kc_key_all, uint32_t *__restrict__ kc_ord_all, uint32_t kc_cap, uint32_t *err_word,
                 const uint64_t *__restrict__ list, const unsigned long long *__restrict__ list_n, uint64_t *gtab, uint32_t *glock,
                 uint32_t g_slices, uint32_t g_slots) {
    __shared__ VoteLds lds;
    __shared__ uint32_t g_H[VG_MAX], g_cnt[VG_MAX], g_ph[VG_MAX];
    __shared__ uint64_t g_id[VG_MAX];
    __shared__ uint32_t s_wsum[12];
    __shared__ Top2 s_top[4];
    __shared__ unsigned long long s_grp;
    __shared__ uint32_t s_slice;
    const uint32_t tid = threadIdx.x, wave = tid >> 6, lane = tid & 63u;
    const uint64_t n_items = list ? (uint64_t) *list_n : v.n * (uint64_t) v.np;
    const uint64_t n_groups = (n_items + vg - 1) / vg;
    const KeyScratch kc = {kc_key_all + (uint64_t) blockIdx.x * kc_cap, kc_ord_all + (uint64_t) blockIdx.x * kc_cap, kc_cap};
    const GlobalPool gp = {gtab, glock, g_slices, g_slots, &s_slice};
    for (;;) {
    if (tid == 0) s_grp = atomicAdd(ticket, 1ull);
    __syncthreads();
    const uint64_t grp = s_grp;
    if (grp >= n_groups) break;
    if (tid < vg) {
        const uint64_t li = grp * vg + tid;
        const uint64_t item = list && li < n_items ? list[li] : li;
        uint32_t H = 0, c = 0, ph = 0;
        uint64_t id = 0;
        if (li < n_items) {
            const ItemId ii = item_decode(item, v);
            ph = ii.iter; id = ii.id;
            if (!(decided && decided[ii.read])) {
                H = ghits[id];
                c = gcnt[id];
                if (H == 0) { LrmPhaseRes z = {0, 0, 0, 0, 0, 0}; v.phase_res[id] = z; }
            }
        }
        g_H[tid] = H; g_cnt[tid] = c; g_id[tid] = id; g_ph[tid] = ph;
    }
    __syncthreads();
    for (uint32_t g = wave; g < vg; g += 4) {
        const uint32_t H = g_H[g];
        if (H == 0 || H > limit1) continue;
        const uint64_t id = g_id[g];
        vote_item_wave<VOTE_U>(ix, v, Item{rec + id * v.cap_q, recq + id * v.cap_q, g_cnt[g], H, g_ph[g], &v.phase_res[id]}, lane, lds.w[wave]);
    }
    __syncthreads();
    for (uint32_t g = 0; g < vg; ++g) {
        const uint32_t H = g_H[g];
        if (H <= limit1) continue;
        const uint64_t id = g_id[g];
        vote_item_block<VOTE_U>(ix, v, Item{rec + id * v.cap_q, recq + id * v.cap_q, g_cnt[g], H, g_ph[g], &v.phase_res[id]}, slots3, limit3, lds.b,
                                s_wsum, s_top, err_word, kc, gp);
        __syncthreads();
    }
    __syncthreads();
    }
}

struct VoteKnobs { uint32_t t3_limit, t3_slots, vg, t1_limit, load; uint64_t *big_tab; };

template <int U>
static void launch_vote_u(lrm_index *idx, lrm_workspace *ws, const LrmVoteLaunch &v, const VoteKnobs &k, hipStream_t stream) {
    LrmDevCounters *c = ws->d_counters;
    const int r = v.round;
    const uint32_t np = (uint32_t) (v.phase_hi - v.phase_lo + 1);
    const uint64_t items = v.n * (uint64_t) np;
    const VoteItems vi = {v.n, (uint32_t) v.seed_len + 1, np, (uint32_t) v.phase_lo, ws->cap_q, v.tbits, k.load, ws->d_phase};
    const uint64_t *list = nullptr;
    const unsigned long long *list_n = nullptr;
    const bool ident32 = idx->view.length < (1ull << 35);
    if (v.mt->vote_fast && ident32) {
        uint64_t fblocks = (items + 4 * FAST_CH - 1) / (4 * FAST_CH);
        if (fblocks > LRM_VOTE_FAST_GRID) fblocks = LRM_VOTE_FAST_GRID;
        hipLaunchKernelGGL(vote_fast_kernel<U>, dim3((uint32_t) fblocks), dim3(256), 0, stream, idx->view, ws->d_rec, ws->d_recq, ws->d_cnt, ws->d_hcount,
                           v.decided, vi, &c->vote_fast_ticket[r], ws->d_redo,
                           &c->vote_redo_n[r], ws->d_big, &c->vote_big_n[r]);
        const uint64_t bblocks = items < 768 ? items : 768;
        hipLaunchKernelGGL(vote_fast_block_kernel<U>, dim3((uint32_t) bblocks), dim3(256), 0, stream, idx->view, ws->d_rec, ws->d_recq, ws->d_cnt, vi,
                           &c->vote_big_ticket[r],
                           (const uint64_t *) ws->d_big, (const unsigned long long *) &c->vote_big_n[r], ws->d_redo, &c->vote_redo_n[r]);
        list = ws->d_redo; list_n = &c->vote_redo_n[r];
    }
    uint64_t vblocks = (items + k.vg - 1) / k.vg;
    if (vblocks > LRM_VOTE_GRID) vblocks = LRM_VOTE_GRID;
    hipLaunchKernelGGL(vote_kernel<U>, dim3((uint32_t) vblocks), dim3(256), 0, stream, idx->view, ws->d_rec, ws->d_recq, ws->d_cnt,
                       ws->d_hcount, v.decided, vi, k.t3_slots, k.t3_limit, k.vg, k.t1_limit,
                       &c->vote_ticket[r], ws->d_kc_key, ws->d_kc_ord, (uint32_t) LRM_VOTE_KC_CAP, ws->d_err, list, list_n, k.big_tab, ws->d_glock,
                       ws->g_slices, ws->g_slots);
}

int lrm_launch_vote(lrm_index *idx, lrm_workspace *ws, const LrmVoteLaunch &v, void *stream_) {
    hipStream_t stream = (hipStream_t) stream_;
    const LrmMapTune &mt = *v.mt;
    VoteKnobs k;
    k.t3_limit = mt.t3_limit ? mt.t3_limit : (uint32_t) T3_LIMIT;
    k.t3_slots = mt.t3_slots >= 8 && mt.t3_slots <= T3_SLOTS ? mt.t3_slots : (uint32_t) T3_SLOTS;
    k.vg = mt.vote_vg >= 1 && mt.vote_vg <= VG_MAX ? mt.vote_vg : VG;
    k.t1_limit = mt.vote_t1 <= T1_LIMIT ? mt.vote_t1 : (uint32_t) T1_LIMIT;
    k.load = mt.vote_load;
    k.big_tab = mt.t3_limit ? nullptr : ws->d_gtab;
    lrm_time_begin(ws, LRM_K_VOTE, stream);
    switch ((int) mt.vote_u) {
        case 2: launch_vote_u<2>(idx, ws, v, k, stream); break;
        case 8: launch_vote_u<8>(idx, ws, v, k, stream); break;
        default: launch_vote_u<4>(idx, ws, v, k, stream); break;
    }
    lrm_time_end(ws, stream);
    return 0;
}
```

### longreadmapper_amd/csrc/workspace.hip

```cpp
#include <hip/hip_runtime.h>
#include <cstring>
#include <new>
#include <vector>
#include "lrm_hip_util.h"
#include "extend_stage.h"

extern "C" void lrm_workspace_free(lrm_workspace *ws) {
    if (!ws) return;
    (void) hipSetDevice(ws->device);
    lrm_dev_free({ws->d_reads2, ws->d_rec, ws->d_phase, ws->d_decided, ws->d_hcount, ws->d_counters, ws->d_recq, ws->d_cnt, ws->d_kc_key,
                  ws->d_kc_ord, ws->d_redo, ws->d_big, ws->d_gtab, ws->d_glock, ws->d_mq_phase});
    lrm_bs_scratch_free(&ws->bs);
    lrm_anchor_scratch_free(ws);
    lrm_split_scratch_free(ws);
    lrm_sec_scratch_free(ws);
    if (ws->h_err) (void) hipHostFree((void *) ws->h_err);
    for (int i = 0; i < LRM_MAX_TIMED; ++i) {
        if (ws->ev_start[i]) (void) hipEventDestroy((hipEvent_t) ws->ev_start[i]);
        if (ws->ev_stop[i]) (void) hipEventDestroy((hipEvent_t) ws->ev_stop[i]);
    }
    delete ws;
}

extern "C" uint64_t lrm_workspace_bytes(const lrm_workspace *ws) { return ws ? ws->bytes : 0; }

extern "C" int lrm_workspace_create(lrm_workspace **out, lrm_index *idx, uint64_t n_max, uint32_t max_len,
                                    uint32_t seed_len, uint32_t thres) {
    return lrm_workspace_create_parts(out, idx, n_max, max_len, seed_len, thres, LRM_WS_SEED | LRM_WS_EXTEND);
}

int lrm_workspace_create_parts(lrm_workspace **out, lrm_index *idx, uint64_t n_max, uint32_t max_len,
                               uint32_t seed_len, uint32_t thres, int parts) {
    if (!out || !idx) { lrm_set_error("null argument"); return -1; }
    if (seed_len < 1 || seed_len > 32) { lrm_set_error("seed_len %u outside [1,32]", seed_len); return -1; }
    if (thres >= (1u << 24)) { lrm_set_error("thres %u >= 2^24 unsupported", thres); return -1; }
    if (n_max == 0) n_max = 1;
    if (lrm_require_device(idx->device)) return -1;
    lrm_workspace *ws = new (std::nothrow) lrm_workspace;
    if (!ws) { lrm_set_error("out of memory"); return -1; }
    memset(ws, 0, sizeof(*ws));
    ws->idx = idx; ws->device = idx->device; ws->n_max = n_max; ws->max_len = max_len;
    ws->seed_len = seed_len; ws->thres = thres;
    ws->P = seed_len + 1;
    uint32_t jl = max_len > seed_len ? max_len - seed_len : 0;
    ws->cap_q = (jl + ws->P - 1) / ws->P;
    if (ws->cap_q == 0) ws->cap_q = 1;
    ws->words_per_read = (uint64_t) max_len / 32 + 2;
    ws->parts = parts;
    {
        const uint64_t hmax = (uint64_t) ws->cap_q * (thres > 1 ? thres - 1 : 1);
        uint64_t gs = 1024;
        while (gs < 2 * hmax && gs < (1ull << 26)) gs <<= 1;
        uint64_t nsl = (256ull << 20) / (gs * 16);
        ws->g_slots = (uint32_t) gs;
        ws->g_slices = (uint32_t) (nsl < 2 ? 2 : nsl > 32 ? 32 : nsl);
    }
    const LrmDevAlloc seed[] = {
        {(void **) &ws->d_reads2, n_max * ws->words_per_read * 8 + 128},
        {(void **) &ws->d_rec, n_max * (uint64_t) ws->P * ws->cap_q * 8},
        {(void **) &ws->d_recq, n_max * (uint64_t) ws->P * ws->cap_q * 4},
        {(void **) &ws->d_cnt, n_max * (uint64_t) ws->P * 4},
        {(void **) &ws->d_kc_key, (uint64_t) LRM_VOTE_GRID * LRM_VOTE_KC_CAP * 8},
        {(void **) &ws->d_kc_ord, (uint64_t) LRM_VOTE_GRID * LRM_VOTE_KC_CAP * 4},
        {(void **) &ws->d_redo, n_max * (uint64_t) ws->P * 8},
        {(void **) &ws->d_big, n_max * (uint64_t) ws->P * 8},
        {(void **) &ws->d_gtab, (uint64_t) ws->g_slices * ws->g_slots * 16},
        {(void **) &ws->d_glock, 64 * 4},
        {(void **) &ws->d_phase, n_max * (uint64_t) ws->P * sizeof(LrmPhaseRes)},
        {(void **) &ws->d_decided, n_max},
        {(void **) &ws->d_hcount, n_max * (uint64_t) ws->P * 4},
    };
    const LrmDevAlloc both[] = {{(void **) &ws->d_counters, sizeof(LrmDevCounters)}};
    if (((parts & LRM_WS_SEED) && lrm_dev_alloc_table(seed, "workspace bytes", &ws->bytes)) ||
        ((parts & (LRM_WS_SEED | LRM_WS_EXTEND)) && lrm_dev_alloc_table(both, "workspace bytes", &ws->bytes))) {
        lrm_workspace_free(ws);
        return -1;
    }
    if ((parts & LRM_WS_EXTEND) && lrm_bs_scratch_alloc(&ws->bs, n_max, max_len, max_len, &ws->bytes)) { lrm_workspace_free(ws); return -1; }
    if (hipMemset(ws->d_counters, 0, sizeof(LrmDevCounters)) != hipSuccess) { lrm_workspace_free(ws); lrm_set_error("memset failed"); return -1; }
    if (ws->d_glock && hipMemset(ws->d_glock, 0, 64 * 4) != hipSuccess) { lrm_workspace_free(ws); lrm_set_error("memset failed"); return -1; }
    {
        void *h = nullptr, *d = nullptr;
        if (hipHostMalloc(&h, 64, hipHostMallocMapped | hipHostMallocCoherent) != hipSuccess ||
            hipHostGetDevicePointer(&d, h, 0) != hipSuccess) {
            if (h) (void) hipHostFree(h);
            lrm_workspace_free(ws);
            lrm_set_error("allocation of the workspace error word failed");
            return -1;
        }
        memset(h, 0, 64);
        ws->h_err = (volatile uint32_t *) h;
        ws->d_err = (uint32_t *) d;
    }
    *out = ws;
    return 0;
}

int lrm_ws_take_error(lrm_workspace *ws) {
    if (!ws || !ws->h_err) return 0;
    const uint32_t e = *ws->h_err;
    if (!e) return 0;
    *ws->h_err = 0;
    if (e & LRM_ERR_VOTE_OVERFLOW)
        lrm_set_error("vote table overflow in the multi-pass tier: results of some phases of an earlier batch on this workspace are invalid");
    else lrm_set_error("device error word 0x%x", e);
    return -2;
}

extern "C" int lrm_workspace_stats(lrm_workspace *ws, lrm_stats *out, void *stream) {
    if (!ws || !out) { lrm_set_error("null argument"); return -1; }
    HIPCHK(hipSetDevice(ws->device));
    LrmDevCounters c;
    HIPCHK(hipMemcpyAsync(&c, ws->d_counters, sizeof(c), hipMemcpyDeviceToHost, (hipStream_t) stream));
    HIPCHK(hipStreamSynchronize((hipStream_t) stream));
    {
        std::vector<uint32_t> hc((size_t) ws->n_last * ws->P);
        if (!hc.empty() && ws->d_hcount) HIPCHK(hipMemcpy(hc.data(), ws->d_hcount, hc.size() * 4, hipMemcpyDeviceToHost));
        else hc.clear();
        uint64_t t2 = 0, t3 = 0;
        for (uint32_t h : hc) { t2 += (h > LRM_VOTE_T1_LIMIT && h <= LRM_VOTE_T3_LIMIT); t3 += (h > LRM_VOTE_T3_LIMIT); }
        out->vote_tier2_items = t2;
        out->vote_tier3_items = t3;
    }
    out->reads_decided_phase0 = c.decided_phase0;
    out->gact_tiles = c.gact_tiles;
    out->vote_redo_items = c.vote_redo_n[0] + c.vote_redo_n[1];
    out->seeds_evaluated = c.seed_traffic[0];
    out->seed_table_lookups = c.seed_traffic[1];
    out->seed_rank_requests = c.seed_traffic[2];
    out->bs_wave_tiles = c.bs_count[LRM_BSC_WAVE_TILES];
    out->bs_pass1_pairs_masked = c.bs_count[LRM_BSC_P1_MASKED];
    out->bs_pass1_pairs_plain = c.bs_count[LRM_BSC_P1_PLAIN];
    out->bs_blocks_full = c.bs_count[LRM_BSC_P2_FULL];
    out->bs_blocks_windowed = c.bs_count[LRM_BSC_P2_WINDOWED];
    out->bs_blocks_skipped = c.bs_count[LRM_BSC_P2_SKIPPED];
    out->bs_refill_rounds = c.bs_count[LRM_BSC_REFILLS];
    return lrm_ws_take_error(ws);
}

extern "C" int lrm_debug_vote_results(lrm_workspace *ws, uint64_t n, uint64_t *out, void *stream) {
    if (!ws || !out || !ws->d_phase) { lrm_set_error("null argument"); return -1; }
    if (n > ws->n_last) { lrm_set_error("the last seed call on this workspace had %llu reads", (unsigned long long) ws->n_last); return -1; }
    HIPCHK(hipSetDevice(ws->device));
    HIPCHK(hipMemcpyAsync(out, ws->d_phase, n * (uint64_t) ws->P * sizeof(LrmPhaseRes), hipMemcpyDeviceToHost, (hipStream_t) stream));
    HIPCHK(hipStreamSynchronize((hipStream_t) stream));
    return 0;
}

void lrm_time_begin(lrm_workspace *ws, int kernel, void *stream) {
    if (!ws || !ws->timing || ws->n_timed >= LRM_MAX_TIMED) return;
    int i = ws->n_timed;
    if (!ws->ev_start[i]) {
        hipEvent_t a, b;
        if (hipEventCreate(&a) != hipSuccess || hipEventCreate(&b) != hipSuccess) return;
        ws->ev_start[i] = a; ws->ev_stop[i] = b;
    }
    ws->ev_kernel[i] = kernel;
    (void) hipEventRecord((hipEvent_t) ws->ev_start[i], (hipStream_t) stream);
}

void lrm_time_end(lrm_workspace *ws, void *stream) {
    if (!ws || !ws->timing || ws->n_timed >= LRM_MAX_TIMED || !ws->ev_stop[ws->n_timed]) return;
    (void) hipEventRecord((hipEvent_t) ws->ev_stop[ws->n_timed], (hipStream_t) stream);
    ws->n_timed++;
}

extern "C" int lrm_workspace_set_counting(lrm_workspace *ws, int enable) {
    if (!ws) { lrm_set_error("null argument"); return -1; }
    ws->counting = enable ? 1 : 0;
    return 0;
}

extern "C" int lrm_workspace_set_timing(lrm_workspace *ws, int enable) {
    if (!ws) { lrm_set_error("null argument"); return -1; }
    ws->timing = enable ? 1 : 0;
    ws->n_timed = 0;
    return 0;
}

extern "C" int lrm_workspace_timing(lrm_workspace *ws, double *ms, uint64_t *launches, void *stream) {
    if (!ws || !ms || !launches) { lrm_set_error("null argument"); return -1; }
    HIPCHK(hipSetDevice(ws->device));
    HIPCHK(hipStreamSynchronize((hipStream_t) stream));
    for (int i = 0; i < ws->n_timed; ++i) {
        float t = 0;
        HIPCHK(hipEventElapsedTime(&t, (hipEvent_t) ws->ev_start[i], (hipEvent_t) ws->ev_stop[i]));
        ms[ws->ev_kernel[i]] += (double) t;
        launches[ws->ev_kernel[i]] += 1;
    }
    ws->n_timed = 0;
    return 0;
}

extern "C" const char *lrm_kernel_name(int k) {
    static const char *names[LRM_K_COUNT] = {"pack2bit_kernel", "seed_search_kernel", "vote_kernel", "decide_kernel",
                                             "locus_resolve_kernel", "revcomp_kernel", "gact_kernel",
                                             "bs_pack_reads_kernel", "gact_bs_kernel"};
    return k >= 0 && k < LRM_K_COUNT ? names[k] : "?";
}
```

### longreadmapper_amd/device.py

```python
import ctypes as C

import numpy as np

from . import capi
from .capi import check, lib
from .records import (ANCHOR_DT, CLIP_DT, DEFAULT_GACT, DEFAULT_SEED_LEN, DEFAULT_THRES, ENTRY_DT, MAPQ_DT, META_DT, N_KERNELS,
                      SECONDARY_DT, SEGMENT_DT, SUMMARY_DT, store_need, units16)


def _records(t, dt):
    return t.cpu().numpy().reshape(-1).view(dt)


def _timing(ws, stream):
    ms = np.zeros(N_KERNELS, dtype=np.float64)
    launches = np.zeros(N_KERNELS, dtype=np.uint64)
    check(lib.lrm_workspace_timing(ws, ms.ctypes.data, launches.ctypes.data, stream), "lrm_workspace_timing")
    return {lib.lrm_kernel_name(i).decode(): (float(ms[i]), int(launches[i])) for i in range(N_KERNELS)}


class DeviceMapper:

    def __init__(self, index, n_max, max_len, seed_len=DEFAULT_SEED_LEN, thres=DEFAULT_THRES, gact=DEFAULT_GACT,
                 device=0, anchored=False, anchor_min_len=0, clip=False, clip_penalty=0, clip_end_bonus=0, split=False,
                 split_min_len=0, seg_cap=None, seg_rows=None, mapq=False, summary=False, md=False, secondary=False, sec_cap=None,
                 sec_min_hits=0, sec_ratio_pct=0):
        import torch
        self.torch = torch
        self.index = index
        self.n_max, self.max_len = n_max, max_len
        self.seed_len, self.thres, self.gact = seed_len, thres, gact
        self.dev = torch.device("cuda", device)
        ws = C.c_void_p()
        check(lib.lrm_workspace_create(C.byref(ws), index.handle, n_max, max_len, seed_len, thres),
              "lrm_workspace_create")
        self.ws = ws
        anchored = bool(anchored or clip)
        self.anchored, self.anchor_min_len = anchored, anchor_min_len
        self.clip_on, self.clip_penalty, self.clip_end_bonus = bool(clip), clip_penalty, clip_end_bonus
        self.store_stride = units16(store_need(max_len, True)) if anchored else store_need(max_len, False)
        t = self._result_tensors(n_max)
        self.best, self.store, self.n_ops = t["best"], t["store"], t["n_ops"]
        self.score, self.meta, self.meta_r = t["score"], t["meta"], t["meta_r"]
        self.anchor = self._record_tensor(n_max, ANCHOR_DT) if anchored else None
        self.clip = self._record_tensor(n_max, CLIP_DT, torch.int32) if clip else None
        self.mapq = self._record_tensor(n_max, MAPQ_DT) if mapq else None
        self.summary = self._record_tensor(n_max, SUMMARY_DT) if summary or md else None
        self.diff_off = torch.zeros(n_max + 1, dtype=torch.int64, device=self.dev) if md else None
        self.diff_events = torch.zeros(1, dtype=torch.int32, device=self.dev) if md else None
        self.sec, self.n_sec = None, 0
        if secondary:
            if not mapq:
                raise capi.LrmError("DeviceMapper: secondary needs mapq")
            cap = self.sec_cap = n_max if sec_cap is None else sec_cap
            k = max(cap, 1)
            self.sec_row_stride = (max_len + 16) // 16 * 16
            self.sec_store_stride = units16(self.store_stride)
            g = self.sec = dict(table=self._record_tensor(k, SECONDARY_DT, torch.int32),
                                rows=torch.zeros((k, self.sec_row_stride), dtype=torch.uint8, device=self.dev),
                                lens=torch.zeros(k, dtype=torch.int32, device=self.dev),
                                rival=self._record_tensor(k, ENTRY_DT, torch.int64),
                                store=torch.zeros((k, self.sec_store_stride), dtype=torch.uint8, device=self.dev),
                                n_ops=torch.zeros(k, dtype=torch.int32, device=self.dev),
                                score=torch.zeros(k, dtype=torch.int32, device=self.dev), meta=self._record_tensor(k, META_DT),
                                meta_r=torch.zeros(k, dtype=torch.int32, device=self.dev))
            if anchored:
                g["anchor"] = self._record_tensor(k, ANCHOR_DT)
            if clip:
                g["clip"] = self._record_tensor(k, CLIP_DT, torch.int32)
            ptr = {name: t.data_ptr() for name, t in g.items()}
            self.sec_dev = capi.SecondaryDev(cap, ptr["table"], ptr["rows"], self.sec_row_stride, ptr["lens"], ptr["rival"], ptr["store"],
                                             self.sec_store_stride, ptr["n_ops"], ptr["score"], ptr["meta"], ptr["meta_r"],
                                             ptr.get("anchor"), ptr.get("clip"))
            self.sec_opt = capi.SecondaryOptions(C.sizeof(capi.SecondaryOptions), sec_min_hits, sec_ratio_pct, int(anchored),
                                                 anchor_min_len, int(bool(clip)), clip_penalty, clip_end_bonus)
        self.split_on, self.split_min_len, self.ws_seg, self.n_seg = bool(split), split_min_len, None, 0
        if split:
            if not clip:
                raise capi.LrmError("DeviceMapper: split needs clip")
            cap = self.seg_cap = 2 * n_max if seg_cap is None else seg_cap
            rows = min(cap, n_max) if seg_rows is None else seg_rows
            if rows:
                wseg = C.c_void_p()
                check(lib.lrm_workspace_create(C.byref(wseg), index.handle, rows, max_len, seed_len, thres), "lrm_workspace_create")
                self.ws_seg = wseg
            k = max(cap, 1)
            self.seg_row_stride = (max_len + 16) // 16 * 16
            g = self.seg = dict(seg=self._record_tensor(k, SEGMENT_DT, torch.int32),
                                rows=torch.zeros((k, self.seg_row_stride), dtype=torch.uint8, device=self.dev),
                                lens=torch.zeros(k, dtype=torch.int32, device=self.dev), **self._result_tensors(k),
                                anchor=self._record_tensor(k, ANCHOR_DT), clip=self._record_tensor(k, CLIP_DT, torch.int32))
            self.split_dev = capi.SplitDev(cap, g["seg"].data_ptr(), g["rows"].data_ptr(), self.seg_row_stride, g["lens"].data_ptr(),
                                           g["best"].data_ptr(), g["store"].data_ptr(), self.store_stride, g["n_ops"].data_ptr(),
                                           g["score"].data_ptr(), g["meta"].data_ptr(), g["meta_r"].data_ptr(),
                                           g["anchor"].data_ptr(), g["clip"].data_ptr())

    def _record_tensor(self, rows, dt, word=None):
        word = word or self.torch.uint8
        return self.torch.zeros((rows, dt.itemsize // word.itemsize), dtype=word, device=self.dev)

    def _result_tensors(self, rows):
        i32 = dict(dtype=self.torch.int32, device=self.dev)
        return dict(best=self._record_tensor(rows, ENTRY_DT, self.torch.int64),
                    store=self.torch.zeros((rows, self.store_stride), dtype=self.torch.uint8, device=self.dev),
                    n_ops=self.torch.zeros(rows, **i32), score=self.torch.zeros(rows, **i32),
                    meta=self._record_tensor(rows, META_DT), meta_r=self.torch.zeros(rows, **i32))

    def workspace_bytes(self):
        return int(lib.lrm_workspace_bytes(self.ws))

    def _stream(self):
        return C.c_void_p(self.torch.cuda.current_stream(self.dev).cuda_stream)

    def seed(self, d_reads, d_lens, n=None):
        n = d_reads.shape[0] if n is None else n
        p = capi.Params(n, self.seed_len, self.thres)
        if self.mapq is not None:
            check(lib.lrm_seed_batch_mapq_dev(self.index.handle, self.ws, d_reads.data_ptr(), d_reads.stride(0),
                                              d_lens.data_ptr(), n, self.max_len, p, self.best.data_ptr(),
                                              self.mapq.data_ptr(), self._stream()), "lrm_seed_batch_mapq_dev")
            return
        check(lib.lrm_seed_batch_dev(self.index.handle, self.ws, d_reads.data_ptr(), d_reads.stride(0),
                                     d_lens.data_ptr(), n, self.max_len, p, self.best.data_ptr(), self._stream()),
              "lrm_seed_batch_dev")

    def mapq_records(self, n):
        assert self.mapq is not None
        return _records(self.mapq[:n], MAPQ_DT)

    def summary_records(self, n):
        assert self.summary is not None
        return _records(self.summary[:n], SUMMARY_DT)

    def diff_records(self, n):
        assert self.diff_off is not None
        off = self.diff_off[:n + 1].cpu().numpy().view(np.uint64)
        return off, self.diff_events[:int(off[n])].cpu().numpy().view(np.uint32)

    def extend(self, d_reads, d_lens, n=None):
        n = d_reads.shape[0] if n is None else n
        self._extend(d_reads, d_lens, n)
        if self.summary is not None:
            check(lib.lrm_aln_summary_dev(self.index.handle, self.store.data_ptr(), self.store_stride, self.n_ops.data_ptr(),
                                          self.score.data_ptr(), self.meta_r.data_ptr(), n, self.summary.data_ptr(),
                                          self._stream()), "lrm_aln_summary_dev")
        if self.diff_off is not None:
            check(lib.lrm_aln_diff_offsets_dev(self.summary.data_ptr(), n, self.diff_off.data_ptr(), self._stream()),
                  "lrm_aln_diff_offsets_dev")
            total = int(self.diff_off[n].item())
            if total > self.diff_events.numel():
                self.diff_events = self.torch.zeros(total, dtype=self.torch.int32, device=self.dev)
            check(lib.lrm_aln_diff_dev(self.index.handle, self.store.data_ptr(), self.store_stride, self.n_ops.data_ptr(),
                                       self.score.data_ptr(), self.meta_r.data_ptr(), self.meta.data_ptr(), n, self.diff_off.data_ptr(),
                                       total, self.diff_events.data_ptr(), self._stream()), "lrm_aln_diff_dev")

    def _extend(self, d_reads, d_lens, n):
        args = (self.index.handle, self.ws, d_reads.data_ptr(), d_reads.stride(0), d_lens.data_ptr(), n, self.max_len,
                self.best.data_ptr(), capi.GactParams(*self.gact), self.store.data_ptr(), self.store_stride, self.n_ops.data_ptr(),
                self.score.data_ptr(), self.meta.data_ptr(), self.meta_r.data_ptr())
        if self.clip_on:
            check(lib.lrm_extend_batch_clipped_dev(*args, self.anchor.data_ptr(), self.anchor_min_len, self.clip_penalty,
                                                   self.clip_end_bonus, self.clip.data_ptr(), self._stream()),
                  "lrm_extend_batch_clipped_dev")
        elif self.anchored:
            check(lib.lrm_extend_batch_anchored_dev(*args, self.anchor.data_ptr(), self.anchor_min_len, self._stream()),
                  "lrm_extend_batch_anchored_dev")
        else:
            check(lib.lrm_extend_batch_dev(*args, self._stream()), "lrm_extend_batch_dev")

    def split(self, d_reads, d_lens, n=None):
        assert self.split_on
        n = d_reads.shape[0] if n is None else n
        k = C.c_uint64()
        rc = lib.lrm_split_batch_dev(self.index.handle, self.ws_seg or self.ws, d_reads.data_ptr(), d_reads.stride(0), d_lens.data_ptr(),
                                     n, self.clip.data_ptr(), capi.Params(n, self.seed_len, self.thres), capi.GactParams(*self.gact),
                                     self.anchor_min_len, self.clip_penalty, self.clip_end_bonus, self.split_min_len,
                                     C.byref(self.split_dev), C.byref(k), self._stream())
        self.n_seg = int(k.value) if rc >= 0 else 0
        if rc < 0:
            raise capi.failure("lrm_split_batch_dev", rc=rc, n_seg=int(k.value))
        return self.n_seg

    def rival(self, d_lens, n, min_hits=0, ratio_pct=0):
        assert self.mapq is not None
        out = self._record_tensor(max(n, 1), ENTRY_DT, self.torch.int64)
        check(lib.lrm_rival_dev(self.index.handle, self.ws, d_lens.data_ptr(), n, capi.Params(n, self.seed_len, self.thres),
                                self.best.data_ptr(), self.mapq.data_ptr(), min_hits, ratio_pct, out.data_ptr(), self._stream()),
              "lrm_rival_dev")
        return out[:n]

    def secondary(self, d_reads, d_lens, n=None, as_sequenced=False):
        assert self.sec is not None
        n = d_reads.shape[0] if n is None else n
        k = C.c_uint64()
        meta, meta_r = (None, None) if as_sequenced else (self.meta.data_ptr(), self.meta_r.data_ptr())
        rc = lib.lrm_secondary_batch_dev(self.index.handle, self.ws, d_reads.data_ptr(), d_reads.stride(0), d_lens.data_ptr(), n,
                                         self.best.data_ptr(), self.mapq.data_ptr(), meta, meta_r,
                                         capi.Params(n, self.seed_len, self.thres), capi.GactParams(*self.gact), C.byref(self.sec_opt),
                                         C.byref(self.sec_dev), C.byref(k), self._stream())
        self.n_sec = int(k.value) if rc >= 0 else 0
        if rc < 0:
            raise capi.failure("lrm_secondary_batch_dev", rc=rc, n_sec=int(k.value))
        return self.n_sec

    def secondary_results(self):
        k = self.n_sec
        h = {"ops" if name == "store" else name: t[:k].cpu().numpy() for name, t in self.sec.items()}
        for name, dt in (("table", SECONDARY_DT), ("rival", ENTRY_DT), ("meta", META_DT), ("anchor", ANCHOR_DT), ("clip", CLIP_DT)):
            if name in h:
                h[name] = h[name].reshape(-1).view(dt)
        h["lens"] = h["lens"].view(np.uint32)
        return h

    def seg_timing(self):
        return _timing(self.ws_seg or self.ws, self._stream())

    def split_results(self):
        k, g = self.n_seg, self.seg
        h = {"ops" if name == "store" else name: t[:k].cpu().numpy() for name, t in g.items()}
        for name, dt in (("seg", SEGMENT_DT), ("best", ENTRY_DT), ("meta", META_DT), ("anchor", ANCHOR_DT), ("clip", CLIP_DT)):
            h[name] = h[name].reshape(-1).view(dt)
        h["lens"] = h["lens"].view(np.uint32)
        return dict(h, is_text=False)

    def stats(self):
        st = capi.Stats()
        check(lib.lrm_workspace_stats(self.ws, C.byref(st), self._stream()), "lrm_workspace_stats")
        return {name: int(getattr(st, name)) for name, _ in capi.Stats._fields_}

    def debug_vote_results(self, n):
        out = np.zeros((n, self.seed_len + 1, 6), dtype=np.uint64)
        check(lib.lrm_debug_vote_results(self.ws, n, out.ctypes.data, self._stream()), "lrm_debug_vote_results")
        return out

    def set_counting(self, enable=True):
        check(lib.lrm_workspace_set_counting(self.ws, int(enable)), "lrm_workspace_set_counting")

    def set_timing(self, enable=True):
        check(lib.lrm_workspace_set_timing(self.ws, int(enable)), "lrm_workspace_set_timing")

    def timing(self):
        return _timing(self.ws, self._stream())

    def results(self, n):
        res = dict(best=_records(self.best[:n], ENTRY_DT), ops=self.store[:n].cpu().numpy(), n_ops=self.n_ops[:n].cpu().numpy(),
                   score=self.score[:n].cpu().numpy(), meta=_records(self.meta[:n], META_DT), meta_r=self.meta_r[:n].cpu().numpy())
        if self.anchored:
            res["anchor"] = _records(self.anchor[:n], ANCHOR_DT)
        if self.clip_on:
            res["clip"] = _records(self.clip[:n], CLIP_DT)
        if self.split_on:
            res["split"] = self.split_results()
        if self.mapq is not None:
            res["mapq"] = self.mapq_records(n)
        if self.summary is not None:
            res["summary"] = self.summary_records(n)
        return res

    def close(self):
        if getattr(self, "ws_seg", None):
            lib.lrm_workspace_free(self.ws_seg)
            self.ws_seg = None
        if self.ws:
            lib.lrm_workspace_free(self.ws)
            self.ws = None

    def __del__(self):
        try:
            self.close()
        except Exception:
            pass
```

Measured before the change: 60.17 Gbp/s.

## Restructure fast vote kernel: wave hit search, packed ranks, prefetched item headers

The fast vote kernel now maps hits to seeds with a wavefront ballot search rather than the generic per-thread loop. When the count and order fit in 32 bits it packs rank keys into 32-bit words, and it decodes items with reciprocal multiplies. Each ticket's decided/hit-count words are prefetched with one lane per item and broadcast via readlane, and unsampled-SA and counting variants are templated out. Opt-in vote counters are added for profiling. These changes add template variants and a new np<32768 launch guard.

```diff
diff --git a/include/lrm_accel.h b/include/lrm_accel.h
--- a/include/lrm_accel.h
+++ b/include/lrm_accel.h
@@ -409,6 +409,12 @@
 int lrm_workspace_set_counting(lrm_workspace *ws, int enable);
 int lrm_workspace_stats(lrm_workspace *ws, lrm_stats *out, void *stream);
 
+#define LRM_N_VOTE_COUNTERS 23
+#define LRM_VOTE_COUNTER_NAMES "items skipped to_block to_exact processed chunks unique_hits cas_extra repeat_items stagings " \
+                               "staged_seeds walks rounds repeat_hits search_iters find_probes list_entries sketch_scans " \
+                               "unsettled_wide unsettled_list unsettled_sketch steps hit_steps"
+int lrm_workspace_vote_counters(lrm_workspace *ws, uint64_t *out, void *stream);
+
 #define LRM_N_KERNELS 9
 int lrm_workspace_set_timing(lrm_workspace *ws, int enable);
 int lrm_workspace_timing(lrm_workspace *ws, double *ms, uint64_t *launches, void *stream);
diff --git a/longreadmapper_amd/capi.py b/longreadmapper_amd/capi.py
--- a/longreadmapper_amd/capi.py
+++ b/longreadmapper_amd/capi.py
@@ -124,6 +124,7 @@
     "lrm_workspace_stats": (C.c_int, [C.c_void_p, C.POINTER(Stats), C.c_void_p]),
     "lrm_debug_vote_results": (C.c_int, [C.c_void_p, C.c_uint64, C.c_void_p, C.c_void_p]),
     "lrm_workspace_set_counting": (C.c_int, [C.c_void_p, C.c_int]),
+    "lrm_workspace_vote_counters": (C.c_int, [C.c_void_p, C.c_void_p, C.c_void_p]),
     "lrm_workspace_set_timing": (C.c_int, [C.c_void_p, C.c_int]),
     "lrm_workspace_timing": (C.c_int, [C.c_void_p, C.c_void_p, C.c_void_p, C.c_void_p]),
     "lrm_kernel_name": (C.c_char_p, [C.c_int]),
diff --git a/longreadmapper_amd/csrc/lrm_internal.h b/longreadmapper_amd/csrc/lrm_internal.h
--- a/longreadmapper_amd/csrc/lrm_internal.h
+++ b/longreadmapper_amd/csrc/lrm_internal.h
@@ -145,10 +145,36 @@
     unsigned long long vote_big_n[2];
     unsigned long long vote_big_ticket[2];
     unsigned long long bs_count[7];
-};
+    unsigned long long vote_count[24];
+};
+enum { LRM_VC_ITEMS = 0,
+       LRM_VC_SKIPPED,
+       LRM_VC_TO_BLOCK,
+       LRM_VC_TO_EXACT,
+       LRM_VC_PROCESSED,
+       LRM_VC_CHUNKS,
+       LRM_VC_UNIQUE_HITS,
+       LRM_VC_CAS_EXTRA,
+       LRM_VC_REPEAT_ITEMS,
+       LRM_VC_STAGINGS,
+       LRM_VC_STAGED_SEEDS,
+       LRM_VC_WALKS,
+       LRM_VC_ROUNDS,
+       LRM_VC_REPEAT_HITS,
+       LRM_VC_SEARCH_ITERS,
+       LRM_VC_FIND_PROBES,
+       LRM_VC_LIST_ENTRIES,
+       LRM_VC_SKETCH_SCANS,
+       LRM_VC_UNSETTLED_WIDE,
+       LRM_VC_UNSETTLED_LIST,
+       LRM_VC_UNSETTLED_SKETCH,
+       LRM_VC_STEPS,
+       LRM_VC_HIT_STEPS,
+       LRM_VC_N };
+static_assert(LRM_VC_N <= 24, "vote_count holds every LRM_VC_* counter");
 enum { LRM_BSC_WAVE_TILES = 0, LRM_BSC_P1_MASKED, LRM_BSC_P1_PLAIN, LRM_BSC_P2_FULL, LRM_BSC_P2_WINDOWED, LRM_BSC_P2_SKIPPED,
        LRM_BSC_REFILLS, LRM_BSC_N };
-static_assert(offsetof(LrmDevCounters, decided_phase0) == 64 && sizeof(LrmDevCounters) == 216, "counters are addressed by the device as laid out here");
+static_assert(offsetof(LrmDevCounters, decided_phase0) == 64 && sizeof(LrmDevCounters) == 216 + 24 * 8, "counters are addressed by the device as laid out here");
 #define LRM_ERR_VOTE_OVERFLOW 1u
 #define LRM_VOTE_T1_LIMIT 192
 #ifndef LRM_VOTE_T3_SLOTS
diff --git a/longreadmapper_amd/csrc/vote_kernels.hip b/longreadmapper_amd/csrc/vote_kernels.hip
--- a/longreadmapper_amd/csrc/vote_kernels.hip
+++ b/longreadmapper_amd/csrc/vote_kernels.hip
@@ -307,22 +307,24 @@
     return id < 0x80000000u ? (uint64_t) id : (0x0FFFFFFF00000000ull | id);
 }
 
-__device__ __forceinline__ uint32_t fast_insert(const FastTable &t, uint32_t id, uint32_t hash) {
+__device__ __forceinline__ uint32_t fast_insert(const FastTable &t, uint32_t id, uint32_t hash, uint32_t *probes = nullptr) {
     uint32_t slot = (uint32_t) (((uint64_t) hash * t.slots) >> 32);
     for (uint32_t probe = 0; probe < t.slots; ++probe) {
         const uint32_t prev = atomicCAS(&t.ident[slot], EMPTY_ID, id);
         if (prev == EMPTY_ID || prev == id) { atomicAdd(&t.count[slot], 1u); return slot; }
         slot = slot + 1 == t.slots ? 0 : slot + 1;
+        if (probes) ++*probes;
     }
     return FAST_NONE;
 }
-__device__ __forceinline__ uint32_t fast_find(const FastTable &t, uint32_t id, uint32_t hash) {
+__device__ __forceinline__ uint32_t fast_find(const FastTable &t, uint32_t id, uint32_t hash, uint32_t *probes = nullptr) {
     uint32_t slot = (uint32_t) (((uint64_t) hash * t.slots) >> 32);
     for (uint32_t probe = 0; probe < t.slots; ++probe) {
         const uint32_t prev = t.ident[slot];
         if (prev == EMPTY_ID) return FAST_NONE;
         if (prev == id) return slot;
         slot = slot + 1 == t.slots ? 0 : slot + 1;
+        if (probes) ++*probes;
     }
     return FAST_NONE;
 }
@@ -334,15 +336,65 @@
 #define FB_LIST 512
 __device__ __forceinline__ uint32_t hit_word(uint32_t slot, uint64_t key) { return (slot << 4) | ((uint32_t) key & 15u); }
 
+#ifndef LRM_VOTE_WAVE_SEARCH
+#define LRM_VOTE_WAVE_SEARCH 1
+#endif
+__device__ __forceinline__ uint32_t wave_seed_of(uint32_t offl, uint32_t h0, uint32_t lane) {
+    const unsigned long long below = __ballot(offl <= h0);
+    unsigned long long inside = __ballot(offl > h0 && offl - h0 < 64u);
+    unsigned long long begins = 0;
+    while (inside) {
+        const int i = (int) __builtin_ctzll(inside);
+        inside &= inside - 1ull;
+        begins |= 1ull << ((uint32_t) __builtin_amdgcn_readlane((int) offl, i) - h0 - 1u);
+    }
+    return (uint32_t) __popcll(below) - 1u + mask_rank(begins);
+}
+template <int U, typename Sink>
+__device__ __forceinline__ void for_each_hit_wave(const LrmIndexView &ix, const Staged &g, uint32_t lane, Sink sink) {
+    const uint32_t offl = lane < g.cnt ? g.off[lane] : 0xFFFFFFFFu;
+    for (uint32_t hb = 0; hb < g.total; hb += 64 * U) {
+        uint64_t v[U];
+        uint32_t ss[U], tt[U];
+#pragma unroll
+        for (int u = 0; u < U; ++u) {
+            const uint32_t h0 = hb + (uint32_t) u * 64, h = h0 + lane;
+            v[u] = 0; ss[u] = 0; tt[u] = 0;
+            if (h0 < g.total) {
+                const uint32_t s = wave_seed_of(offl, h0, lane);
+                if (h < g.total) {
+                    ss[u] = s;
+                    tt[u] = h - g.off[s];
+                    v[u] = sa_locate(ix, (g.srec[s] & ((1ull << 40) - 1ull)) + tt[u]);
+                }
+            }
+        }
+#pragma unroll
+        for (int u = 0; u < U; ++u) {
+            const uint32_t h = hb + (uint32_t) u * 64 + lane;
+            const bool live = h < g.total;
+            uint64_t key = 0;
+            uint32_t order = 0;
+            if (live) {
+                const uint32_t q = g.sq[ss[u]];
+                key = v[u] - (uint64_t) (g.iter + q * g.P);
+                order = (q << g.tbits) | tt[u];
+            }
+            sink(live, h, key, order);
+        }
+    }
+}
+
 template <int NT, int VOTE_U>
 __device__ __forceinline__ void fast_hits(const LrmIndexView &ix, const FastTable &t, const Staged &g, uint32_t *sketch, uint32_t sk_mask,
-                                          uint32_t tid, uint64_t *list, uint32_t cap, uint32_t &n_list, uint32_t *list_n, bool &wide) {
-    for_each_hit<NT, VOTE_U>(ix, g, tid, [&](bool live, uint32_t, uint64_t key, uint32_t order) __attribute__((always_inline)) {
-        uint32_t hw = FAST_NONE, oinv = 0;
+                                          uint32_t tid, uint64_t *list, uint32_t cap, uint32_t &n_list, uint32_t *list_n, bool &wide,
+                                          uint32_t *taps = nullptr) {
+    auto sink = [&](bool live, uint32_t, uint64_t key, uint32_t order) __attribute__((always_inline)) {
+        uint32_t hw = FAST_NONE, oinv = 0, probes = 0;
         if (live) {
             const uint32_t hash = bucket_hash(key >> 4);
             wide |= key_wide(key);
-            const uint32_t slot = fast_find(t, (uint32_t) (key >> 4), hash);
+            const uint32_t slot = fast_find(t, (uint32_t) (key >> 4), hash, taps ? &probes : nullptr);
             if (slot != FAST_NONE) {
                 atomicAdd(&t.count[slot], 1u);
                 hw = hit_word(slot, key);
@@ -353,6 +405,7 @@
             }
         }
         const unsigned long long bm = __ballot(hw != FAST_NONE);
+        if (taps) { taps[0] += wave_max_u32(probes); taps[1] += __ballot(live) != 0 && bm != 0; }
         if (bm) {
             uint32_t base;
             if (NT == 64) { base = n_list; n_list += (uint32_t) __popcll(bm); }
@@ -366,10 +419,28 @@
                 if (i < cap) list[i] = ((uint64_t) oinv << 32) | hw;
             }
         }
-    });
-}
-
-struct RankTop { uint64_t r; uint32_t s; };
+    };
+    if constexpr (NT == 64 && LRM_VOTE_WAVE_SEARCH) for_each_hit_wave<VOTE_U>(ix, g, tid, sink);
+    else for_each_hit<NT, VOTE_U>(ix, g, tid, sink);
+}
+
+static_assert(T1_LIMIT * 16 < (1 << 12), "a count of the wavefront form fits 12 bits");
+template <bool PACKED> struct RankForm;
+template <> struct RankForm<false> {
+    typedef uint64_t R;
+    static __device__ __forceinline__ R make(uint32_t count, uint32_t oinv, uint32_t) { return ((uint64_t) count << 32) | oinv; }
+    static __device__ __forceinline__ uint32_t val(R r, uint32_t) { return (uint32_t) (r >> 32); }
+    static __device__ __forceinline__ uint32_t first(R r, uint32_t) { return 0xFFFFFFFFu - (uint32_t) r; }
+};
+template <> struct RankForm<true> {
+    typedef uint32_t R;
+    static __device__ __forceinline__ uint32_t mask(uint32_t ob) { return (1u << ob) - 1u; }
+    static __device__ __forceinline__ R make(uint32_t count, uint32_t oinv, uint32_t ob) { return (count << ob) | (oinv & mask(ob)); }
+    static __device__ __forceinline__ uint32_t val(R r, uint32_t ob) { return r >> ob; }
+    static __device__ __forceinline__ uint32_t first(R r, uint32_t ob) { return ~r & mask(ob); }
+};
+template <typename R> struct RankTopT { R r; uint32_t s; };
+typedef RankTopT<uint64_t> RankTop;
 __device__ __forceinline__ RankTop wave_top_rank(const RankTop &x) {
     const uint32_t hi = (uint32_t) (x.r >> 32), lo = (uint32_t) x.r;
     const uint32_t mh = wave_max_u32(hi);
@@ -382,9 +453,19 @@
     }
     return w;
 }
-template <int N>
-__device__ __forceinline__ RankTop lane_top_rank(const uint64_t (&hr)[N], const uint32_t (&hw)[N], uint32_t skip) {
-    RankTop b = {0, 0};
+__device__ __forceinline__ RankTopT<uint32_t> wave_top_rank(const RankTopT<uint32_t> &x) {
+    const uint32_t m = wave_max_u32(x.r);
+    RankTopT<uint32_t> w = {0, 0};
+    if (m) {
+        const unsigned long long b = __ballot(x.r == m);
+        w.r = m;
+        w.s = (uint32_t) __builtin_amdgcn_readlane((int) x.s, (int) __builtin_ctzll(b));
+    }
+    return w;
+}
+template <typename R, int N>
+__device__ __forceinline__ RankTopT<R> lane_top_rank(const R (&hr)[N], const uint32_t (&hw)[N], uint32_t skip) {
+    RankTopT<R> b = {0, 0};
 #pragma unroll
     for (int k = 0; k < N; ++k) {
         const uint32_t s = hw[k] >> 4;
@@ -392,8 +473,8 @@
     }
     return b;
 }
-template <int N>
-__device__ __forceinline__ uint32_t lane_low4_mask(const uint64_t (&hr)[N], const uint32_t (&hw)[N], const RankTop &a, const RankTop &b) {
+template <typename R, int N>
+__device__ __forceinline__ uint32_t lane_low4_mask(const R (&hr)[N], const uint32_t (&hw)[N], const RankTopT<R> &a, const RankTopT<R> &b) {
     uint32_t m = 0;
 #pragma unroll
     for (int k = 0; k < N; ++k) {
@@ -403,19 +484,20 @@
     }
     return m;
 }
-__device__ __forceinline__ TopEntry fast_entry(const FastTable &t, const RankTop &w, uint32_t mask16) {
+template <typename F>
+__device__ __forceinline__ TopEntry fast_entry(const FastTable &t, const RankTopT<typename F::R> &w, uint32_t ob, uint32_t mask16) {
     TopEntry e = {0, 0, 0, 0};
     if (w.r) {
         e.bucket = bucket_of_ident(t.ident[w.s]);
         e.key = (e.bucket << 4) | (uint32_t) (__clz((int) mask16) - 16);
-        e.val = (uint32_t) (w.r >> 32); e.first = 0xFFFFFFFFu - (uint32_t) w.r;
+        e.val = F::val(w.r, ob); e.first = F::first(w.r, ob);
     }
     return e;
 }
 
-template <int NT, int NL, int N>
-__device__ __forceinline__ void list_ranks(const FastTable &t, const uint64_t *list, uint32_t n_list, uint32_t cap, uint32_t tid,
-                                           uint64_t (&hr)[N], uint32_t (&hw)[N]) {
+template <int NT, int NL, typename F, int N>
+__device__ __forceinline__ void list_ranks(const FastTable &t, const uint64_t *list, uint32_t n_list, uint32_t cap, uint32_t tid, uint32_t ob,
+                                           typename F::R (&hr)[N], uint32_t (&hw)[N]) {
 #pragma unroll
     for (int l = 0; l < NL; ++l) {
         const uint32_t i = (uint32_t) l * NT + tid;
@@ -423,7 +505,7 @@
         if (i < n_list && i < cap) {
             const uint64_t x = list[i];
             hw[N - NL + l] = (uint32_t) x;
-            hr[N - NL + l] = ((uint64_t) t.count[(uint32_t) x >> 4] << 32) | (x >> 32);
+            hr[N - NL + l] = F::make(t.count[(uint32_t) x >> 4], (uint32_t) (x >> 32), ob);
         }
     }
 }
@@ -455,33 +537,63 @@
 #define LRM_VOTE_FAST_WAVES (LRM_VOTE_FAST_GRID / 256)
 #endif
 #define FAST_CH 16
-template <int VOTE_U>
+#ifndef LRM_VOTE_STAGE_JOIN
+#define LRM_VOTE_STAGE_JOIN 64
+#endif
+#define FAST_STAGE_JOIN LRM_VOTE_STAGE_JOIN
+static_assert(FAST_STAGE_JOIN >= 0 && FAST_STAGE_JOIN <= 64, "the staging arrays hold 64 seeds");
+struct FastGeom { uint32_t ob, load_inv, np_inv, pad; uint64_t np_inv64; };
+static_assert(FB_LIMIT < 0xFFFF, "a ticket's item word holds every survivor count the fast kernels take");
+template <int VOTE_U, bool PACKED, bool COUNT, bool SAMPLED>
 __global__ __launch_bounds__(256) __attribute__((amdgpu_waves_per_eu(LRM_VOTE_FAST_WAVES, LRM_VOTE_FAST_WAVES)))
 void vote_fast_kernel(LrmIndexView ix, const uint64_t *__restrict__ rec, const uint32_t *__restrict__ recq, const uint32_t *__restrict__ gcnt,
-                      const uint32_t *__restrict__ ghits, const uint8_t *__restrict__ decided, VoteItems v, unsigned long long *ticket, uint64_t *__restrict__ redo, unsigned long long *redo_n,
-                      uint64_t *__restrict__ big, unsigned long long *big_n) {
+                      const uint32_t *__restrict__ ghits, const uint8_t *__restrict__ decided, VoteItems v, FastGeom fg, unsigned long long *ticket,
+                      uint64_t *__restrict__ redo, unsigned long long *redo_n, uint64_t *__restrict__ big, unsigned long long *big_n,
+                      LrmDevCounters *counters) {
+    typedef RankForm<PACKED> F;
+    typedef typename F::R R;
+    if (!SAMPLED) ix.sa_shift = 0;
     __shared__ FastLds lds[4];
     const uint32_t lane = threadIdx.x & 63u;
     FastLds &L = lds[threadIdx.x >> 6];
     const uint64_t n_items = v.n * (uint64_t) v.np;
     constexpr int NU = (T1_LIMIT + 63) / 64;
     constexpr int NL = (FAST_LIST + 63) / 64;
+    static_assert(FAST_CH <= 64, "one lane per item of a ticket");
+    uint32_t nc[LRM_VC_N] = {};
     for (;;) {
         unsigned long long base = 0;
         if (lane == 0) base = atomicAdd(ticket, (unsigned long long) FAST_CH);
         base = ((unsigned long long) (uint32_t) __builtin_amdgcn_readfirstlane((int) (uint32_t) (base >> 32)) << 32) |
                (uint32_t) __builtin_amdgcn_readfirstlane((int) (uint32_t) base);
         if (base >= n_items) break;
-        ItemId ii = item_decode(base, v);
+        ItemId ii;
+        ii.read = fg.np_inv64 ? __umul64hi(base, fg.np_inv64) : base;
+        ii.iter = v.phase_lo + (uint32_t) (base - ii.read * v.np);
+        uint32_t hc = 0;
+        {
+            const uint32_t o = ii.iter - v.phase_lo + lane, dr = fg.np_inv ? __umulhi(o, fg.np_inv) : o;
+            if (lane < FAST_CH && base + lane < n_items) {
+                const uint64_t rd = ii.read + dr;
+                const uint64_t lid = rd * (uint64_t) v.P + v.phase_lo + (o - dr * v.np);
+                if (decided && decided[rd]) hc = FAST_NONE;
+                else {
+                    const uint32_t h = ghits[lid], c = gcnt[lid];
+                    hc = (h ? 0x10000u : 0u) | (c < 0xFFFFu ? c : 0xFFFFu);
+                }
+            }
+        }
         for (uint32_t it = 0; it < FAST_CH && base + it < n_items; ++it, ++ii.iter) {
             if (ii.iter == v.phase_lo + v.np) { ii.iter = v.phase_lo; ++ii.read; }
             const uint64_t item = base + it;
             const uint32_t iter = ii.iter;
             const uint64_t id = ii.read * (uint64_t) v.P + iter;
-            if (decided && decided[ii.read]) continue;
-            const uint32_t H = ghits[id], cnt = gcnt[id];
-            if (H == 0) {
+            const uint32_t hci = (uint32_t) __builtin_amdgcn_readlane((int) hc, (int) it), cnt = hci & 0xFFFFu;
+            if (COUNT) nc[LRM_VC_ITEMS]++;
+            if (hci == FAST_NONE) { if (COUNT) nc[LRM_VC_SKIPPED]++; continue; }
+            if ((hci >> 16) == 0) {
                 if (lane == 0) { LrmPhaseRes z = {0, 0, 0, 0, 0, 0}; v.phase_res[id] = z; }
+                if (COUNT) nc[LRM_VC_SKIPPED]++;
                 continue;
             }
             if (cnt > (uint32_t) T1_LIMIT) {
@@ -489,9 +601,13 @@
                     if (cnt <= (uint32_t) FB_LIMIT) big[atomicAdd(big_n, 1ull)] = item;
                     else redo[atomicAdd(redo_n, 1ull)] = item;
                 }
+                if (COUNT) { if (cnt <= (uint32_t) FB_LIMIT) nc[LRM_VC_TO_BLOCK]++; else nc[LRM_VC_TO_EXACT]++; }
                 continue;
             }
-            const FastTable t = {L.ident, L.count, table_slots_for(cnt, v.load, T1_SLOTS)};
+            if (COUNT) nc[LRM_VC_PROCESSED]++;
+            const uint32_t nch = (cnt + 63u) >> 6;
+            const uint32_t eff = ((cnt * fg.load_inv) >> 16) + 64;
+            const FastTable t = {L.ident, L.count, eff < (uint32_t) T1_SLOTS ? eff : (uint32_t) T1_SLOTS};
             uint64_t e[NU], sv[NU];
             uint32_t qq[NU];
             const uint64_t *irec = rec + id * v.cap_q;
@@ -499,16 +615,22 @@
 #pragma unroll
             for (int u = 0; u < NU; ++u) {
                 const uint32_t s = (uint32_t) u * 64 + lane;
-                e[u] = s < cnt ? irec[s] : 0ull;
-                qq[u] = s < cnt ? iq[s] : 0u;
+                e[u] = 0ull; qq[u] = 0u;
+                if (u == 0 || (uint32_t) u < nch) {
+                    e[u] = s < cnt ? irec[s] : 0ull;
+                    qq[u] = s < cnt ? iq[s] : 0u;
+                }
             }
             table_clear<64>(t, lane);
             unsigned long long any_big = 0;
 #pragma unroll
             for (int u = 0; u < NU; ++u) {
-                const uint32_t rr = (uint32_t) (e[u] >> 40);
-                sv[u] = rr == 1 ? sa_of_unique(ix, e[u]) : 0ull;
-                any_big |= __ballot(rr > 1);
+                sv[u] = 0ull;
+                if (u == 0 || (uint32_t) u < nch) {
+                    const uint32_t rr = (uint32_t) (e[u] >> 40);
+                    sv[u] = rr == 1 ? sa_of_unique(ix, e[u]) : 0ull;
+                    any_big |= __ballot(rr > 1);
+                }
             }
             if (any_big) {
 #pragma unroll
@@ -516,52 +638,102 @@
             }
             __builtin_amdgcn_fence(__ATOMIC_RELEASE, "wavefront");
             __builtin_amdgcn_wave_barrier();
-            uint64_t hr[NU + NL];
+            R hr[NU + NL];
             uint32_t hw[NU + NL];
             bool wide = false;
 #pragma unroll
             for (int u = 0; u < NU; ++u) {
                 hw[u] = FAST_NONE;
-                if ((uint32_t) (e[u] >> 40) == 1) {
-                    const uint64_t key = sv[u] - (uint64_t) (iter + qq[u] * v.P);
-                    wide |= key_wide(key);
-                    const uint32_t slot = fast_insert(t, (uint32_t) (key >> 4), bucket_hash(key >> 4));
-                    if (slot != FAST_NONE) hw[u] = hit_word(slot, key);
+                if (u == 0 || (uint32_t) u < nch) {
+                    const bool uniq = (uint32_t) (e[u] >> 40) == 1;
+                    uint32_t probes = 0;
+                    if (uniq) {
+                        const uint64_t key = sv[u] - (uint64_t) (iter + qq[u] * v.P);
+                        wide |= key_wide(key);
+                        const uint32_t slot = fast_insert(t, (uint32_t) (key >> 4), bucket_hash(key >> 4), COUNT ? &probes : nullptr);
+                        if (slot != FAST_NONE) hw[u] = hit_word(slot, key);
+                    }
+                    if (COUNT) {
+                        nc[LRM_VC_CHUNKS]++;
+                        nc[LRM_VC_UNIQUE_HITS] += (uint32_t) __popcll(__ballot(uniq));
+                        nc[LRM_VC_CAS_EXTRA] += wave_max_u32(probes);
+                    }
                 }
             }
             __builtin_amdgcn_fence(__ATOMIC_ACQ_REL, "wavefront");
             __builtin_amdgcn_wave_barrier();
             uint32_t n_list = 0;
             if (any_big) {
-#pragma unroll
-                for (int u = 0; u < NU; ++u) {
-                    if (__ballot((uint32_t) (e[u] >> 40) > 1) == 0) continue;
-                    const WaveStage st = stage_repeats_wave(L.off, L.srec, L.sq, e[u], qq[u], WaveStage{0, 0}, lane);
-                    fast_hits<64, VOTE_U>(ix, t, Staged{L.off, L.srec, L.sq, st.n, st.hits, iter, v.P, v.tbits}, L.sketch, 2 * FAST_SK_WORDS - 1, lane,
-                                          L.list, (uint32_t) FAST_LIST, n_list, nullptr, wide);
-                    __builtin_amdgcn_fence(__ATOMIC_ACQ_REL, "wavefront");
-                    __builtin_amdgcn_wave_barrier();
+                uint32_t next = 0;
+                do {
+                    WaveStage st = {0, 0};
+                    bool full = false;
+#pragma unroll
+                    for (int u = 0; u < NU; ++u) {
+                        if (full || (uint32_t) u < next || (uint32_t) u >= nch) continue;
+                        const uint32_t nrep = (uint32_t) __popcll(__ballot((uint32_t) (e[u] >> 40) > 1));
+                        if (st.n && nrep && st.n + nrep > (uint32_t) FAST_STAGE_JOIN) { full = true; continue; }
+                        next = (uint32_t) u + 1;
+                        if (nrep == 0) continue;
+                        st = stage_repeats_wave(L.off, L.srec, L.sq, e[u], qq[u], st, lane);
+                        if (COUNT) { nc[LRM_VC_STAGINGS]++; nc[LRM_VC_STAGED_SEEDS] += nrep; }
+                    }
+                    if (st.n) {
+                        uint32_t taps[2] = {0, 0};
+                        fast_hits<64, VOTE_U>(ix, t, Staged{L.off, L.srec, L.sq, st.n, st.hits, iter, v.P, v.tbits}, L.sketch, 2 * FAST_SK_WORDS - 1, lane,
+                                              L.list, (uint32_t) FAST_LIST, n_list, nullptr, wide, COUNT ? taps : nullptr);
+                        __builtin_amdgcn_fence(__ATOMIC_ACQ_REL, "wavefront");
+                        __builtin_amdgcn_wave_barrier();
+                        if (COUNT) {
+                            nc[LRM_VC_WALKS]++;
+                            nc[LRM_VC_ROUNDS] += (st.hits + 64u * VOTE_U - 1) / (64u * VOTE_U);
+                            nc[LRM_VC_REPEAT_HITS] += st.hits;
+                            nc[LRM_VC_SEARCH_ITERS] += ((st.hits + 63u) >> 6) * (st.n > 1 ? 32u - (uint32_t) __builtin_clz(st.n - 1) : 0u);
+                            nc[LRM_VC_FIND_PROBES] += taps[0];
+                            nc[LRM_VC_STEPS] += (st.hits + 63u) >> 6;
+                            nc[LRM_VC_HIT_STEPS] += taps[1];
+                        }
+                    }
+                } while (next < nch);
+            }
+            bool lost = wide;
+#pragma unroll
+            for (int u = 0; u < NU; ++u) {
+                hr[u] = 0;
+                if (u == 0 || (uint32_t) u < nch) {
+                    const bool uniq = (uint32_t) (e[u] >> 40) == 1;
+                    lost |= uniq && hw[u] == FAST_NONE;
+                    if (uniq && hw[u] != FAST_NONE) hr[u] = F::make(t.count[hw[u] >> 4], 0xFFFFFFFFu - (qq[u] << v.tbits), fg.ob);
                 }
             }
-            bool lost = wide;
-#pragma unroll
-            for (int u = 0; u < NU; ++u) {
-                const bool uniq = (uint32_t) (e[u] >> 40) == 1;
-                lost |= uniq && hw[u] == FAST_NONE;
-                hr[u] = uniq && hw[u] != FAST_NONE ? ((uint64_t) t.count[hw[u] >> 4] << 32) | (0xFFFFFFFFu - (qq[u] << v.tbits)) : 0ull;
-            }
-            list_ranks<64, NL>(t, L.list, n_list, (uint32_t) FAST_LIST, lane, hr, hw);
-            const RankTop a = wave_top_rank(lane_top_rank(hr, hw, FAST_NONE));
-            const RankTop b = wave_top_rank(lane_top_rank(hr, hw, a.r ? a.s : FAST_NONE));
+            list_ranks<64, NL, F>(t, L.list, n_list, (uint32_t) FAST_LIST, lane, fg.ob, hr, hw);
+            const RankTopT<R> a = wave_top_rank(lane_top_rank(hr, hw, FAST_NONE));
+            const RankTopT<R> b = wave_top_rank(lane_top_rank(hr, hw, a.r ? a.s : FAST_NONE));
             const uint32_t lowm = wave_or_u32(lane_low4_mask(hr, hw, a, b));
-            bool settled = n_list <= (uint32_t) FAST_LIST && __ballot(lost) == 0;
-            if (any_big) settled = settled && sketch_max<64, FAST_SK_WORDS>(L.sketch, lane) < (uint32_t) (b.r >> 32);
+            const bool any_lost = __ballot(lost) != 0;
+            bool settled = n_list <= (uint32_t) FAST_LIST && !any_lost;
+            bool sk_ok = true;
+            if (any_big) sk_ok = sketch_max<64, FAST_SK_WORDS>(L.sketch, lane) < F::val(b.r, fg.ob);
+            settled = settled && sk_ok;
             if (lane == 0) {
-                if (settled) write_phase(&v.phase_res[id], PhaseTop{fast_entry(t, a, lowm >> 16), fast_entry(t, b, lowm & 0xffffu)});
+                if (settled) write_phase(&v.phase_res[id], PhaseTop{fast_entry<F>(t, a, fg.ob, lowm >> 16), fast_entry<F>(t, b, fg.ob, lowm & 0xffffu)});
                 else redo[atomicAdd(redo_n, 1ull)] = item;
             }
+            if (COUNT) {
+                nc[LRM_VC_LIST_ENTRIES] += n_list;
+                if (any_big) { nc[LRM_VC_REPEAT_ITEMS]++; nc[LRM_VC_SKETCH_SCANS]++; }
+                if (any_lost) nc[LRM_VC_UNSETTLED_WIDE]++;
+                else if (n_list > (uint32_t) FAST_LIST) nc[LRM_VC_UNSETTLED_LIST]++;
+                else if (!sk_ok) nc[LRM_VC_UNSETTLED_SKETCH]++;
+            }
             __builtin_amdgcn_wave_barrier();
         }
+    }
+    if (COUNT && lane < LRM_VC_N) {
+        uint32_t x = 0;
+#pragma unroll
+        for (int k = 0; k < LRM_VC_N; ++k) x = lane == (uint32_t) k ? nc[k] : x;
+        atomicAdd(&counters->vote_count[lane], (unsigned long long) x);
     }
 }
 
@@ -647,7 +819,7 @@
 #pragma unroll
         for (int k = 0; k < NU; ++k)
             hr[k] = hw[k] != FAST_NONE ? ((uint64_t) t.count[hw[k] >> 4] << 32) | ho[k] : 0ull;
-        list_ranks<256, NL>(t, L.list, n_list, (uint32_t) FB_LIST, tid, hr, hw);
+        list_ranks<256, NL, RankForm<false>>(t, L.list, n_list, (uint32_t) FB_LIST, tid, 0u, hr, hw);
         const RankTop wa = wave_top_rank(lane_top_rank(hr, hw, FAST_NONE));
         if (lane == 0) s_rk[0][wave] = wa;
         __syncthreads();
@@ -664,7 +836,7 @@
             uint32_t M = 0, lm = 0;
             for (int x = 0; x < 4; ++x) { M = s_m[x] > M ? s_m[x] : M; lm |= s_or[x]; }
             const bool settled = all_ok && n_list <= (uint32_t) FB_LIST && (!block_big || M < (uint32_t) (b.r >> 32));
-            if (settled) write_phase(&v.phase_res[id], PhaseTop{fast_entry(t, a, lm >> 16), fast_entry(t, b, lm & 0xffffu)});
+            if (settled) write_phase(&v.phase_res[id], PhaseTop{fast_entry<RankForm<false>>(t, a, 0u, lm >> 16), fast_entry<RankForm<false>>(t, b, 0u, lm & 0xffffu)});
             else redo[atomicAdd(redo_n, 1ull)] = item;
         }
         __syncthreads();
@@ -746,12 +918,22 @@
     const uint64_t *list = nullptr;
     const unsigned long long *list_n = nullptr;
     const bool ident32 = idx->view.length < (1ull << 35);
-    if (v.mt->vote_fast && ident32) {
+    if (v.mt->vote_fast && ident32 && np < 32768u) {
         uint64_t fblocks = (items + 4 * FAST_CH - 1) / (4 * FAST_CH);
         if (fblocks > LRM_VOTE_FAST_GRID) fblocks = LRM_VOTE_FAST_GRID;
-        hipLaunchKernelGGL(vote_fast_kernel<U>, dim3((uint32_t) fblocks), dim3(256), 0, stream, idx->view, ws->d_rec, ws->d_recq, ws->d_cnt, ws->d_hcount,
-                           v.decided, vi, &c->vote_fast_ticket[r], ws->d_redo,
-                           &c->vote_redo_n[r], ws->d_big, &c->vote_big_n[r]);
+        uint32_t ob = v.tbits;
+        while (ob < 32 && ((uint64_t) (ws->cap_q - 1) >> (ob - v.tbits)) != 0) ++ob;
+        const bool packed = ob + 12 <= 32;
+        const uint32_t load = k.load ? k.load : 100u;
+        const FastGeom fg = {packed ? ob : 0u, (100u << 16) / load + 1u, np > 1 ? (uint32_t) ((1ull << 32) / np) + 1u : 0u, 0u,
+                             np > 1 ? ~0ull / np + 1ull : 0ull};
+        const bool sampled = idx->view.sa_shift != 0;
+        auto fk = ws->counting ? (packed ? vote_fast_kernel<U, true, true, true> : vote_fast_kernel<U, false, true, true>)
+                  : sampled ? (packed ? vote_fast_kernel<U, true, false, true> : vote_fast_kernel<U, false, false, true>)
+                            : (packed ? vote_fast_kernel<U, true, false, false> : vote_fast_kernel<U, false, false, false>);
+        hipLaunchKernelGGL(fk, dim3((uint32_t) fblocks), dim3(256), 0, stream, idx->view, ws->d_rec, ws->d_recq, ws->d_cnt, ws->d_hcount,
+                           v.decided, vi, fg, &c->vote_fast_ticket[r], ws->d_redo,
+                           &c->vote_redo_n[r], ws->d_big, &c->vote_big_n[r], c);
         const uint64_t bblocks = items < 768 ? items : 768;
         hipLaunchKernelGGL(vote_fast_block_kernel<U>, dim3((uint32_t) bblocks), dim3(256), 0, stream, idx->view, ws->d_rec, ws->d_recq, ws->d_cnt, vi,
                            &c->vote_big_ticket[r],
diff --git a/longreadmapper_amd/csrc/workspace.hip b/longreadmapper_amd/csrc/workspace.hip
--- a/longreadmapper_amd/csrc/workspace.hip
+++ b/longreadmapper_amd/csrc/workspace.hip
@@ -138,6 +138,17 @@
     return lrm_ws_take_error(ws);
 }
 
+static_assert(LRM_N_VOTE_COUNTERS == LRM_VC_N, "the header's counter names are the LRM_VC_* of lrm_internal.h");
+extern "C" int lrm_workspace_vote_counters(lrm_workspace *ws, uint64_t *out, void *stream) {
+    if (!ws || !out) { lrm_set_error("null argument"); return -1; }
+    HIPCHK(hipSetDevice(ws->device));
+    LrmDevCounters c;
+    HIPCHK(hipMemcpyAsync(&c, ws->d_counters, sizeof(c), hipMemcpyDeviceToHost, (hipStream_t) stream));
+    HIPCHK(hipStreamSynchronize((hipStream_t) stream));
+    for (int k = 0; k < LRM_VC_N; ++k) out[k] = c.vote_count[k];
+    return 0;
+}
+
 extern "C" int lrm_debug_vote_results(lrm_workspace *ws, uint64_t n, uint64_t *out, void *stream) {
     if (!ws || !out || !ws->d_phase) { lrm_set_error("null argument"); return -1; }
     if (n > ws->n_last) { lrm_set_error("the last seed call on this workspace had %llu reads", (unsigned long long) ws->n_last); return -1; }
diff --git a/longreadmapper_amd/device.py b/longreadmapper_amd/device.py
--- a/longreadmapper_amd/device.py
+++ b/longreadmapper_amd/device.py
@@ -6,6 +6,11 @@
 from .capi import check, lib
 from .records import (ANCHOR_DT, CLIP_DT, DEFAULT_GACT, DEFAULT_SEED_LEN, DEFAULT_THRES, ENTRY_DT, MAPQ_DT, META_DT, N_KERNELS,
                       SECONDARY_DT, SEGMENT_DT, SUMMARY_DT, store_need, units16)
+
+
+VOTE_COUNTERS = ("items", "skipped", "to_block", "to_exact", "processed", "chunks", "unique_hits", "cas_extra", "repeat_items",
+                 "stagings", "staged_seeds", "walks", "rounds", "repeat_hits", "search_iters", "find_probes", "list_entries",
+                 "sketch_scans", "unsettled_wide", "unsettled_list", "unsettled_sketch", "steps", "hit_steps")
 
 
 def _records(t, dt):
@@ -233,6 +238,11 @@
         check(lib.lrm_debug_vote_results(self.ws, n, out.ctypes.data, self._stream()), "lrm_debug_vote_results")
         return out
 
+    def vote_counters(self):
+        out = np.zeros(len(VOTE_COUNTERS), dtype=np.uint64)
+        check(lib.lrm_workspace_vote_counters(self.ws, out.ctypes.data, self._stream()), "lrm_workspace_vote_counters")
+        return dict(zip(VOTE_COUNTERS, (int(x) for x in out)))
+
     def set_counting(self, enable=True):
         check(lib.lrm_workspace_set_counting(self.ws, int(enable)), "lrm_workspace_set_counting")
 
```

New measurement: 60.10 Gbp/s. No clear change (-0.1%).
